# kimerein/sabatinilab-glm

Measured on NVIDIA B200. Metric: cv_model_fits_per_sec, higher is better.
Workload: dtype f64

## Files before the change

### sabatinilab-glm_b200/csrc/gram_tc.cu

```cuda
#include <cuda.h>

#include <algorithm>
#include <vector>

#include <stdlib.h>

#include "common.cuh"

namespace sglm {

constexpr int TC_SMAX = 8;
constexpr int TC_BK = 128;
constexpr int TC_BM = 256;
constexpr int TC_BN = 256;
constexpr int TC_STAGES = 3;
constexpr int TC_THREADS = 192;
constexpr int TC_MAX_KB_PER_SEG = 2048;
constexpr uint32_t TC_STAGE_BYTES = (TC_BM + TC_BN) * TC_BK;
constexpr int TC_LEAD = 64;
constexpr int TC_FAR = 1024;

__device__ __forceinline__ double z_value(const double *X, long long ldx, const double *Y, long long ldy,
                                          int C, int n_y, long long t, int c) {
    if (c < C) return X[t * ldx + c];
    if (c < C + n_y) return Y[t * ldy + (c - C)];
    return 1.0;
}

__global__ void __launch_bounds__(256)
tc_colmax_kernel(const double *__restrict__ X, long long ldx, const double *__restrict__ Y, long long ldy,
                 int C, int n_y, long long T, const double *__restrict__ rs,
                 unsigned long long *__restrict__ colmax_bits, int *__restrict__ col_lsb) {
    const int n_aug = C + n_y + 1;
    const int c = blockIdx.x * 256 + threadIdx.x;
    if (c >= n_aug) return;
    const long long rows_per = (T + gridDim.y - 1) / gridDim.y;
    const long long t0 = (long long)blockIdx.y * rows_per, t1 = min(T, t0 + rows_per);
    double m = 0.0;
    bool bad = false;
    int lsb = 0x7fffffff;
    for (long long t = t0; t < t1; ++t) {
        const double v = fabs(z_value(X, ldx, Y, ldy, C, n_y, t, c) * (rs ? rs[t] : 1.0));
        bad |= !(v <= 1.7976931348623157e308);
        m = fmax(m, v);
        const long long bits = __double_as_longlong(v);
        const int e = (int)(bits >> 52);
        const long long frac = bits & 0xfffffffffffffLL;
        if (e > 0) lsb = min(lsb, e - 1075 + __ffsll(frac | (1LL << 52)) - 1);
        else if (frac) lsb = min(lsb, -1074 + __ffsll(frac) - 1);
    }
    if (bad) m = __longlong_as_double(0x7ff8000000000000LL);
    atomicMax(colmax_bits + c, (unsigned long long)__double_as_longlong(m));
    atomicMin(col_lsb + c, lsb);
}

__device__ __forceinline__ int digits_needed(double z, int E) {
    double r = scalbn(z, -E);
    int need = 0;
    r *= 64.0;
#pragma unroll
    for (int k = 1; k <= TC_SMAX; ++k) {
        if (r == 0.0) break;
        const double d = rint(r);
        if (d != 0.0) need = k;
        r = (r - d) * 128.0;
    }
    if (r != 0.0) need = TC_SMAX;
    return need;
}

__global__ void __launch_bounds__(256)
tc_digits_kernel(const double *__restrict__ X, long long ldx, const double *__restrict__ Y, long long ldy,
                 int C, int n_y, long long T, const double *__restrict__ rs, const int *__restrict__ colE,
                 int *__restrict__ colS) {
    const int n_aug = C + n_y + 1;
    const int c = blockIdx.x * 256 + threadIdx.x;
    if (c >= n_aug) return;
    const long long rows_per = (T + gridDim.y - 1) / gridDim.y;
    const long long t0 = (long long)blockIdx.y * rows_per, t1 = min(T, t0 + rows_per);
    const int E = colE[c];
    int need = 1;
    for (long long t = t0; t < t1 && need < TC_SMAX; ++t)
        need = max(need, digits_needed(z_value(X, ldx, Y, ldy, C, n_y, t, c) * (rs ? rs[t] : 1.0), E));
    atomicMax(colS + c, need);
}

__global__ void tc_exponent_kernel(const unsigned long long *__restrict__ colmax_bits, int n_aug, int max_planes,
                                   int *__restrict__ colE, int *__restrict__ colS, int *__restrict__ flag) {
    const int c = blockIdx.x * blockDim.x + threadIdx.x;
    if (c >= n_aug) return;
    const double m = __longlong_as_double((long long)colmax_bits[c]);
    if (!(m <= 1.7976931348623157e308)) { atomicOr(flag, 1); colE[c] = 0; colS[c] = 1; return; }
    const int E = (m == 0.0) ? 0 : ilogb(m) + 1;
    colE[c] = E;
    const int lsb = colS[c];
    int need = 1;
    if (m != 0.0) {
        const int span = E - 6 - lsb;
        if (span > 0) need = 1 + (span + 6) / 7;
    }
    colS[c] = min(need, max_planes);
}

__global__ void __launch_bounds__(256)
tc_slice_kernel(const double *__restrict__ X, long long ldx, const double *__restrict__ Y, long long ldy,
                int C, int n_y, const double *__restrict__ rs, const long long *__restrict__ rows, long long n_pos,
                const int *__restrict__ colE, const int *__restrict__ colS, const int *__restrict__ plane_row,
                int8_t *__restrict__ At, long long ld_at, long long n_ident) {
    __shared__ __align__(16) double tile[32][130];
    const int n_aug = C + n_y + 1;
    const long long p0 = (long long)blockIdx.x * 128;
    const int c0 = blockIdx.y * 32;
    const int tid = threadIdx.x;
    __shared__ long long srow[128];
    if (tid < 128) srow[tid] = (p0 + tid < n_pos) ? (rows ? rows[p0 + tid] : (p0 + tid < n_ident ? p0 + tid : -1)) : -1;
    __syncthreads();
    {
        const int cc = tid & 31, c = c0 + cc;
        double v[16];
#pragma unroll
        for (int k = 0; k < 16; ++k) {
            const long long t = srow[(tid >> 5) + 8 * k];
            v[k] = (t >= 0 && c < n_aug) ? z_value(X, ldx, Y, ldy, C, n_y, t, c) * (rs ? rs[t] : 1.0) : 0.0;
        }
#pragma unroll
        for (int k = 0; k < 16; ++k) tile[cc][(tid >> 5) + 8 * k] = v[k];
    }
    __syncthreads();
    const int pq = tid & 31, cg = tid >> 5;
    const long long p = p0 + 4 * pq;
    if (p >= n_pos) return;
#pragma unroll 1
    for (int cc = cg * 4; cc < cg * 4 + 4; ++cc) {
        const int c = c0 + cc;
        if (c >= n_aug) break;
        const int S = colS[c], E = colE[c];
        const double2 v01 = *reinterpret_cast<const double2 *>(&tile[cc][4 * pq]);
        const double2 v23 = *reinterpret_cast<const double2 *>(&tile[cc][4 * pq + 2]);
        double r0, r1, r2, r3;
        if (E > -900 && E < 900) {
            const double sc = __longlong_as_double((long long)(1023 + 6 - E) << 52);
            r0 = v01.x * sc; r1 = v01.y * sc; r2 = v23.x * sc; r3 = v23.y * sc;
        } else {
            r0 = scalbn(v01.x, -E) * 64.0; r1 = scalbn(v01.y, -E) * 64.0;
            r2 = scalbn(v23.x, -E) * 64.0; r3 = scalbn(v23.y, -E) * 64.0;
        }
        for (int k = 1; k <= S; ++k) {
            const double d0 = rint(r0), d1 = rint(r1), d2 = rint(r2), d3 = rint(r3);
            r0 = (r0 - d0) * 128.0; r1 = (r1 - d1) * 128.0; r2 = (r2 - d2) * 128.0; r3 = (r3 - d3) * 128.0;
            const unsigned pack = ((unsigned)(int)d0 & 0xffu) | (((unsigned)(int)d1 & 0xffu) << 8) |
                                  (((unsigned)(int)d2 & 0xffu) << 16) | (((unsigned)(int)d3 & 0xffu) << 24);
            *reinterpret_cast<unsigned *>(At + (long long)plane_row[c * TC_SMAX + (k - 1)] * ld_at + p) = pack;
        }
    }
}

constexpr int TC_EXP_ROWS = 256;
constexpr int TC_EXP_POS = 512;
__global__ void __launch_bounds__(256)
tc_expand_kernel(const int8_t *__restrict__ Bt, long long ld_bt, const long long *__restrict__ rows, long long n_pos,
                 const int2 *__restrict__ map, int n_at_rows, int8_t *__restrict__ At, long long ld_at) {
    __shared__ long long srow[TC_EXP_POS];
    const int tid = threadIdx.x;
    const long long p0 = (long long)blockIdx.x * TC_EXP_POS;
    for (int i = tid; i < TC_EXP_POS; i += 256) srow[i] = (p0 + i < n_pos) ? rows[p0 + i] : -1;
    __syncthreads();
    const int pq = tid & 31, rl = tid >> 5;
    const long long p = p0 + 16 * pq;
    if (p >= n_pos) return;
    const long long r0 = srow[16 * pq], r15 = srow[16 * pq + 15];
    const bool contig = r0 >= 0 && r15 == r0 + 15;
    const int r_end = min(n_at_rows, (int)(blockIdx.y + 1) * TC_EXP_ROWS);
    for (int r = blockIdx.y * TC_EXP_ROWS + rl; r < r_end; r += 8) {
        const int2 m = map[r];
        if (m.x < 0) continue;
        const int8_t *src = Bt + (long long)m.x * ld_bt + m.y;
        uint4 out;
        if (contig) {
            const unsigned long long a = (unsigned long long)(src + r0);
            const unsigned *w = reinterpret_cast<const unsigned *>(a & ~3ull);
            const unsigned sh = (unsigned)(a & 3ull) * 8u;
            const unsigned w0 = __ldg(w), w1 = __ldg(w + 1), w2 = __ldg(w + 2), w3 = __ldg(w + 3);
            const unsigned w4 = sh ? __ldg(w + 4) : 0u;
            out = make_uint4(__funnelshift_r(w0, w1, sh), __funnelshift_r(w1, w2, sh), __funnelshift_r(w2, w3, sh),
                             __funnelshift_r(w3, w4, sh));
        } else {
            unsigned q[4];
#pragma unroll
            for (int j = 0; j < 4; ++j) {
                unsigned v = 0u;
#pragma unroll
                for (int b = 0; b < 4; ++b) {
                    const long long rr = srow[16 * pq + 4 * j + b];
                    if (rr >= 0) v |= (unsigned)(unsigned char)__ldg(src + rr) << (8 * b);
                }
                q[j] = v;
            }
            out = make_uint4(q[0], q[1], q[2], q[3]);
        }
        *reinterpret_cast<uint4 *>(At + (long long)r * ld_at + p) = out;
    }
}

__device__ __forceinline__ uint32_t smem_u32(const void *p) { return (uint32_t)__cvta_generic_to_shared(p); }

__device__ __forceinline__ void mbar_init(uint64_t *bar, uint32_t count) {
    asm volatile("mbarrier.init.shared::cta.b64 [%0], %1;" ::"r"(smem_u32(bar)), "r"(count));
}
__device__ __forceinline__ void mbar_expect_tx(uint64_t *bar, uint32_t bytes) {
    asm volatile("mbarrier.arrive.expect_tx.shared::cta.b64 _, [%0], %1;" ::"r"(smem_u32(bar)), "r"(bytes) : "memory");
}
__device__ __forceinline__ void mbar_arrive(uint64_t *bar) {
    asm volatile("mbarrier.arrive.shared::cta.b64 _, [%0];" ::"r"(smem_u32(bar)) : "memory");
}
__device__ __forceinline__ void mbar_wait(uint64_t *bar, uint32_t parity) {
    const uint32_t addr = smem_u32(bar);
    const long long t_start = clock64();
    while (true) {
        uint32_t done;
        asm volatile(
            "{\n\t.reg .pred p;\n\t"
            "mbarrier.try_wait.parity.shared::cta.b64 p, [%1], %2;\n\t"
            "selp.b32 %0, 1, 0, p;\n\t}"
            : "=r"(done)
            : "r"(addr), "r"(parity)
            : "memory");
        if (done) return;
        if (clock64() - t_start > 4000000000LL) { asm volatile("trap;"); }
    }
}
__device__ __forceinline__ void tma_load_2d(void *dst, const CUtensorMap *tmap, uint64_t *bar, int c0, int c1) {
    asm volatile(
        "cp.async.bulk.tensor.2d.shared::cluster.global.mbarrier::complete_tx::bytes [%0], [%1, {%3, %4}], [%2];"
        ::"r"(smem_u32(dst)), "l"((uint64_t)tmap), "r"(smem_u32(bar)), "r"(c0), "r"(c1)
        : "memory");
}
__device__ __forceinline__ void tma_load_2d_mc(void *dst, const CUtensorMap *tmap, uint64_t *bar, int c0, int c1, uint16_t mask) {
    asm volatile(
        "cp.async.bulk.tensor.2d.shared::cluster.global.mbarrier::complete_tx::bytes.multicast::cluster [%0], [%1, {%3, %4}], [%2], %5;"
        ::"r"(smem_u32(dst)), "l"((uint64_t)tmap), "r"(smem_u32(bar)), "r"(c0), "r"(c1), "h"(mask)
        : "memory");
}
__device__ __forceinline__ void tc_commit_mc(uint64_t *bar, uint16_t mask) {
    asm volatile("tcgen05.commit.cta_group::1.mbarrier::arrive::one.shared::cluster.multicast::cluster.b64 [%0], %1;"
                 ::"r"(smem_u32(bar)), "h"(mask) : "memory");
}
__device__ __forceinline__ void tc_cluster_sync() {
    asm volatile("barrier.cluster.arrive.release.aligned;\n\tbarrier.cluster.wait.acquire.aligned;" ::: "memory");
}
__device__ __forceinline__ void tc_fence_before() { asm volatile("tcgen05.fence::before_thread_sync;" ::: "memory"); }
__device__ __forceinline__ void tc_fence_after() { asm volatile("tcgen05.fence::after_thread_sync;" ::: "memory"); }
__device__ __forceinline__ void tc_commit(uint64_t *bar) {
    asm volatile("tcgen05.commit.cta_group::1.mbarrier::arrive::one.shared::cluster.b64 [%0];" ::"r"(smem_u32(bar)) : "memory");
}
__device__ __forceinline__ void tc_mma_i8(uint32_t tmem_d, uint64_t desc_a, uint64_t desc_b, uint32_t idesc, uint32_t accumulate) {
    asm volatile(
        "{\n\t.reg .pred p;\n\t"
        "setp.ne.b32 p, %4, 0;\n\t"
        "tcgen05.mma.cta_group::1.kind::i8 [%0], %1, %2, %3, p;\n\t}"
        ::"r"(tmem_d), "l"(desc_a), "l"(desc_b), "r"(idesc), "r"(accumulate)
        : "memory");
}
__device__ __forceinline__ uint64_t umma_desc_k_sw128(uint32_t smem_addr) {
    uint64_t d = 0;
    d |= (uint64_t)((smem_addr >> 4) & 0x3FFF);
    d |= (uint64_t)1 << 16;
    d |= (uint64_t)(1024 >> 4) << 32;
    d |= (uint64_t)1 << 46;
    d |= (uint64_t)2 << 61;
    return d;
}
__host__ __device__ constexpr uint32_t tc_idesc_i8() {
    return (2u << 4) | (1u << 7) | (1u << 10) | ((uint32_t)(TC_BN >> 3) << 17) | ((uint32_t)(128 >> 4) << 24);
}

struct TcSeg { int kb0, n_kb, set, first; };

__global__ void __launch_bounds__(TC_THREADS, 1)
tc_gram_i8_kernel(const __grid_constant__ CUtensorMap tmap, const int2 *__restrict__ tiles, int n_tiles,
                  int n_parts, const TcSeg *__restrict__ segs, int n_segs, long long *__restrict__ SG, long long S,
                  int *__restrict__ prog, const int2 *__restrict__ pairs, int n_pairs) {
    extern __shared__ __align__(1024) uint8_t tc_smem[];
    uint8_t *base = (uint8_t *)(((uintptr_t)tc_smem + 1023) & ~(uintptr_t)1023);
    uint8_t *sA = base;
    uint8_t *sB = base + TC_STAGES * TC_BM * TC_BK;
    uint64_t *bars = (uint64_t *)(base + TC_STAGES * TC_STAGE_BYTES);
    uint64_t *full = bars, *empty = bars + TC_STAGES, *tmem_full = bars + 2 * TC_STAGES, *tmem_empty = tmem_full + 1;
    uint32_t *tmem_slot = (uint32_t *)(tmem_empty + 1);

    const int warp = threadIdx.x >> 5, lane = threadIdx.x & 31;
    const int item = blockIdx.x;
    const int rank = item & 1;
    const int2 pr = pairs[(item >> 1) % n_pairs];
    const int part = (item >> 1) / n_pairs;
    const bool paired = pr.y >= 0;
    const int my_tile = rank == 0 ? pr.x : pr.y;
    const int2 tile = tiles[my_tile >= 0 ? my_tile : pr.x];
    const int m0 = tile.x * TC_BM, n0 = tile.y * TC_BN;
    (void)n_tiles;
    long long total_kb = 0;
    for (int sgi = 0; sgi < n_segs; ++sgi) total_kb += segs[sgi].n_kb;
    const long long part_lo = total_kb * part / n_parts, part_hi = total_kb * (part + 1) / n_parts;
    auto seg_range = [&](const TcSeg &sg, long long before, int &lo, int &hi) {
        const long long a = max(part_lo, before), b = min(part_hi, before + sg.n_kb);
        lo = sg.kb0 + (int)(a - before);
        hi = (b > a) ? sg.kb0 + (int)(b - before) : lo;
    };

    if (threadIdx.x == 0) {
        for (int s = 0; s < TC_STAGES; ++s) { mbar_init(full + s, 1); mbar_init(empty + s, paired ? 2 : 1); }
        mbar_init(tmem_full, 1);
        mbar_init(tmem_empty, 4);
        asm volatile("fence.mbarrier_init.release.cluster;" ::: "memory");
    }
    if (warp == 1) {
        asm volatile("tcgen05.alloc.cta_group::1.sync.aligned.shared::cta.b32 [%0], %1;" ::"r"(smem_u32(tmem_slot)), "r"(512));
        asm volatile("tcgen05.relinquish_alloc_permit.cta_group::1.sync.aligned;" ::);
    }
    tc_fence_before();
    __syncthreads();
    tc_cluster_sync();
    tc_fence_after();
    const uint32_t tmem_acc = *tmem_slot;
    const uint16_t mc_mask = paired ? (uint16_t)3 : (uint16_t)(1u << rank);

    if (my_tile < 0) {
        if (prog != nullptr && threadIdx.x == 0)
            asm volatile("st.relaxed.gpu.global.s32 [%0], %1;" ::"l"(prog + item), "r"(0x7fffffff) : "memory");
    } else if (warp == 0) {
        int it = 0;
        long long before = 0;
        for (int sgi = 0; sgi < n_segs; ++sgi) {
            int lo, hi;
            seg_range(segs[sgi], before, lo, hi);
            before += segs[sgi].n_kb;
            for (int kb = lo; kb < hi; ++kb, ++it) {
                if (prog != nullptr && (it & 31) == 0) {
                    __syncwarp();
                    if (lane == 0) asm volatile("st.relaxed.gpu.global.s32 [%0], %1;" ::"l"(prog + item), "r"(it) : "memory");
                    const int *grp = prog + (long long)part * 2 * n_pairs;
                    const long long t_start = clock64();
                    while (true) {
                        int behind = 0;
                        for (int j = lane; j < 2 * n_pairs; j += 32) {
                            int v;
                            asm volatile("ld.relaxed.gpu.global.s32 %0, [%1];" : "=r"(v) : "l"(grp + j) : "memory");
                            const int d = it - v;
                            if (v >= 0 && d > TC_LEAD && d <= TC_FAR) behind = 1;
                        }
                        if (!__any_sync(0xffffffffu, behind)) break;
                        __nanosleep(500);
                        if (clock64() - t_start > 4000000000LL) { asm volatile("trap;"); }
                    }
                }
                if (lane == 0) {
                    const int st = it % TC_STAGES;
                    const uint32_t ph = (it / TC_STAGES) & 1;
                    mbar_wait(empty + st, ph ^ 1);
                    mbar_expect_tx(full + st, TC_STAGE_BYTES);
                    const int kc = kb * TC_BK;
                    uint8_t *a = sA + st * TC_BM * TC_BK, *bq = sB + st * TC_BN * TC_BK;
                    if (paired) {
                        tma_load_2d_mc(a + rank * 128 * TC_BK, &tmap, full + st, kc, m0 + 128 * rank, mc_mask);
                    } else {
                        tma_load_2d(a, &tmap, full + st, kc, m0);
                        tma_load_2d(a + 128 * TC_BK, &tmap, full + st, kc, m0 + 128);
                    }
                    tma_load_2d(bq, &tmap, full + st, kc, n0);
                    tma_load_2d(bq + 128 * TC_BK, &tmap, full + st, kc, n0 + 128);
                }
            }
        }
        __syncwarp();
        if (prog != nullptr && lane == 0)
            asm volatile("st.relaxed.gpu.global.s32 [%0], %1;" ::"l"(prog + item), "r"(0x7fffffff) : "memory");
    } else if (warp == 1) {
        if (lane == 0) {
            constexpr uint32_t idesc = tc_idesc_i8();
            int it = 0, drained = 0;
            long long before = 0;
            for (int sgi = 0; sgi < n_segs; ++sgi) {
                int lo, hi;
                seg_range(segs[sgi], before, lo, hi);
                before += segs[sgi].n_kb;
                if (hi <= lo) continue;
                if (drained > 0) { mbar_wait(tmem_empty, (drained - 1) & 1); tc_fence_after(); }
                for (int kb = lo; kb < hi; ++kb, ++it) {
                    const int st = it % TC_STAGES;
                    const uint32_t ph = (it / TC_STAGES) & 1;
                    mbar_wait(full + st, ph);
                    tc_fence_after();
                    const uint64_t da0 = umma_desc_k_sw128(smem_u32(sA + st * TC_BM * TC_BK));
                    const uint64_t da1 = umma_desc_k_sw128(smem_u32(sA + st * TC_BM * TC_BK + 128 * TC_BK));
                    const uint64_t db = umma_desc_k_sw128(smem_u32(sB + st * TC_BN * TC_BK));
#pragma unroll
                    for (int k = 0; k < TC_BK / 32; ++k) {
                        const uint32_t accflag = ((kb - lo) | k) ? 1u : 0u;
                        tc_mma_i8(tmem_acc, da0 + (uint64_t)(k * 2), db + (uint64_t)(k * 2), idesc, accflag);
                        tc_mma_i8(tmem_acc + 256u, da1 + (uint64_t)(k * 2), db + (uint64_t)(k * 2), idesc, accflag);
                    }
                    if (paired) tc_commit_mc(empty + st, mc_mask);
                    else tc_commit(empty + st);
                }
                tc_commit(tmem_full);
                ++drained;
            }
        }
    } else {
        const int q = warp & 3;
        const int row = q * 32 + lane;
        int drained = 0;
        long long before = 0;
        for (int sgi = 0; sgi < n_segs; ++sgi) {
            const TcSeg sg = segs[sgi];
            int lo, hi;
            seg_range(sg, before, lo, hi);
            before += sg.n_kb;
            if (hi <= lo) continue;
            mbar_wait(tmem_full, drained & 1);
            tc_fence_after();
#pragma unroll 1
            for (int half = 0; half < 2; ++half) {
                unsigned long long *out = reinterpret_cast<unsigned long long *>(
                    SG + ((long long)sg.set * S + (m0 + half * 128 + row)) * S + n0);
#pragma unroll 1
                for (int ch = 0; ch < TC_BN / 32; ++ch) {
                    uint32_t v[32];
                    const uint32_t taddr = tmem_acc + ((uint32_t)(q * 32) << 16) + (uint32_t)(half * 256 + ch * 32);
                    asm volatile(
                        "tcgen05.ld.sync.aligned.32x32b.x32.b32 "
                        "{%0, %1, %2, %3, %4, %5, %6, %7, %8, %9, %10, %11, %12, %13, %14, %15, "
                        "%16, %17, %18, %19, %20, %21, %22, %23, %24, %25, %26, %27, %28, %29, %30, %31}, [%32];"
                        : "=r"(v[0]), "=r"(v[1]), "=r"(v[2]), "=r"(v[3]), "=r"(v[4]), "=r"(v[5]), "=r"(v[6]), "=r"(v[7]),
                          "=r"(v[8]), "=r"(v[9]), "=r"(v[10]), "=r"(v[11]), "=r"(v[12]), "=r"(v[13]), "=r"(v[14]), "=r"(v[15]),
                          "=r"(v[16]), "=r"(v[17]), "=r"(v[18]), "=r"(v[19]), "=r"(v[20]), "=r"(v[21]), "=r"(v[22]), "=r"(v[23]),
                          "=r"(v[24]), "=r"(v[25]), "=r"(v[26]), "=r"(v[27]), "=r"(v[28]), "=r"(v[29]), "=r"(v[30]), "=r"(v[31])
                        : "r"(taddr));
                    asm volatile("tcgen05.wait::ld.sync.aligned;" ::: "memory");
#pragma unroll
                    for (int j = 0; j < 32; ++j) {
                        const long long x = (long long)(int)v[j];
                        if (x != 0) atomicAdd(out + ch * 32 + j, (unsigned long long)x);
                    }
                }
            }
            tc_fence_before();
            __syncwarp();
            if (lane == 0) mbar_arrive(tmem_empty);
            ++drained;
        }
    }
    tc_fence_before();
    __syncthreads();
    tc_cluster_sync();
    if (warp == 1) {
        tc_fence_after();
        asm volatile("tcgen05.dealloc.cta_group::1.sync.aligned.b32 %0, %1;" ::"r"(tmem_acc), "r"(512));
    }
}

__global__ void __launch_bounds__(TC_THREADS, 1)
tc_mma_probe_kernel(int iters) {
    extern __shared__ __align__(1024) uint8_t tc_smem[];
    uint8_t *base = (uint8_t *)(((uintptr_t)tc_smem + 1023) & ~(uintptr_t)1023);
    uint64_t *bars = (uint64_t *)(base + TC_STAGE_BYTES);
    uint32_t *tmem_slot = (uint32_t *)(bars + 2);
    const int warp = threadIdx.x >> 5, lane = threadIdx.x & 31;
    for (int i = threadIdx.x; i < (int)(TC_STAGE_BYTES / 4); i += TC_THREADS) ((uint32_t *)base)[i] = 0x01010101u * (i & 3);
    if (threadIdx.x == 0) { mbar_init(bars, 1); asm volatile("fence.mbarrier_init.release.cluster;" ::: "memory"); }
    if (warp == 1) {
        asm volatile("tcgen05.alloc.cta_group::1.sync.aligned.shared::cta.b32 [%0], %1;" ::"r"(smem_u32(tmem_slot)), "r"(512));
        asm volatile("tcgen05.relinquish_alloc_permit.cta_group::1.sync.aligned;" ::);
    }
    asm volatile("fence.proxy.async.shared::cta;" ::: "memory");
    tc_fence_before();
    __syncthreads();
    tc_fence_after();
    const uint32_t tmem_acc = *tmem_slot;
    if (warp == 1 && lane == 0) {
        constexpr uint32_t idesc = tc_idesc_i8();
        const uint64_t da0 = umma_desc_k_sw128(smem_u32(base));
        const uint64_t da1 = umma_desc_k_sw128(smem_u32(base + 128 * TC_BK));
        const uint64_t db = umma_desc_k_sw128(smem_u32(base + TC_BM * TC_BK));
        for (int it = 0; it < iters; ++it) {
#pragma unroll
            for (int k = 0; k < TC_BK / 32; ++k) {
                tc_mma_i8(tmem_acc, da0 + (uint64_t)(k * 2), db + (uint64_t)(k * 2), idesc, (it | k) ? 1u : 0u);
                tc_mma_i8(tmem_acc + 256u, da1 + (uint64_t)(k * 2), db + (uint64_t)(k * 2), idesc, (it | k) ? 1u : 0u);
            }
        }
        tc_commit(bars);
        mbar_wait(bars, 0);
    }
    tc_fence_before();
    __syncthreads();
    if (warp == 1) {
        tc_fence_after();
        asm volatile("tcgen05.dealloc.cta_group::1.sync.aligned.b32 %0, %1;" ::"r"(tmem_acc), "r"(512));
    }
}

__global__ void __launch_bounds__(256)
tc_gram_i8_check_kernel(const int8_t *__restrict__ At, long long ld_at, const int2 *__restrict__ tiles,
                        const TcSeg *__restrict__ segs, int n_segs, long long *__restrict__ SG, long long S) {
    const int2 tile = tiles[blockIdx.x];
    const int m0 = tile.x * TC_BM, n0 = tile.y * TC_BN;
    for (int e = threadIdx.x; e < TC_BM * TC_BN; e += 256) {
        const int m = m0 + e / TC_BN, n = n0 + e % TC_BN;
        const int *a = reinterpret_cast<const int *>(At + (long long)m * ld_at);
        const int *b = reinterpret_cast<const int *>(At + (long long)n * ld_at);
        for (int sgi = 0; sgi < n_segs; ++sgi) {
            const TcSeg sg = segs[sgi];
            long long acc = 0;
            const long long i0 = (long long)sg.kb0 * (TC_BK / 4), i1 = i0 + (long long)sg.n_kb * (TC_BK / 4);
            int part = 0;
            for (long long i = i0; i < i1; ++i) {
                part = __dp4a(a[i], b[i], part);
                if ((i & 1023) == 1023) { acc += part; part = 0; }
            }
            acc += part;
            SG[((long long)sg.set * S + m) * S + n] += acc;
        }
    }
}

constexpr int TC_SUM_OUT = 8;
constexpr int TC_SUM_CELLS = 256;
__global__ void __launch_bounds__(256)
tc_zero_tiles_kernel(long long *__restrict__ SG, long long S, const int2 *__restrict__ tiles) {
    const int2 tile = tiles[blockIdx.x];
    long long *base = SG + (long long)blockIdx.y * S * S + (long long)tile.x * TC_BM * S + (long long)tile.y * TC_BN;
    for (int e = threadIdx.x; e < TC_BM * TC_BN / 2; e += 256) {
        const int r = e / (TC_BN / 2), c2 = e % (TC_BN / 2);
        reinterpret_cast<longlong2 *>(base + (long long)r * S)[c2] = make_longlong2(0, 0);
    }
}

__global__ void __launch_bounds__(256)
tc_cell_sum_kernel(const long long *__restrict__ SG, long long S, const int2 *__restrict__ tiles, int n_tiles, int n_cells,
                   const int *__restrict__ member, int n_out, long long *__restrict__ SGout) {
    __shared__ unsigned smask[TC_SUM_CELLS];
    const long long n_elem = S * S;
    const long long n_pairs = (long long)n_tiles * (TC_BM * TC_BN / 2);
    for (int o0 = 0; o0 < n_out; o0 += TC_SUM_OUT) {
        __syncthreads();
        for (int c = threadIdx.x; c < n_cells && c < TC_SUM_CELLS; c += 256) {
            unsigned m = 0;
            for (int k = 0; k < TC_SUM_OUT && o0 + k < n_out; ++k)
                if (member[(o0 + k) * n_cells + c]) m |= 1u << k;
            smask[c] = m;
        }
        __syncthreads();
        for (long long t = (long long)blockIdx.x * 256 + threadIdx.x; t < n_pairs; t += (long long)gridDim.x * 256) {
            const int2 tile = tiles[t / (TC_BM * TC_BN / 2)];
            const int w = (int)(t % (TC_BM * TC_BN / 2));
            const long long e = ((long long)tile.x * TC_BM + w / (TC_BN / 2)) * S + (long long)tile.y * TC_BN + 2 * (w % (TC_BN / 2));
            const bool two = true;
            long long a0[TC_SUM_OUT], a1[TC_SUM_OUT];
#pragma unroll
            for (int k = 0; k < TC_SUM_OUT; ++k) { a0[k] = 0; a1[k] = 0; }
#pragma unroll 4
            for (int c = 0; c < n_cells; ++c) {
                const long long *src = SG + (long long)c * n_elem + e;
                long long v0, v1 = 0;
                if (two) { const longlong2 v = *reinterpret_cast<const longlong2 *>(src); v0 = v.x; v1 = v.y; }
                else v0 = src[0];
                const unsigned m = smask[c];
#pragma unroll
                for (int k = 0; k < TC_SUM_OUT; ++k)
                    if ((m >> k) & 1u) { a0[k] += v0; a1[k] += v1; }
            }
#pragma unroll
            for (int k = 0; k < TC_SUM_OUT; ++k)
                if (o0 + k < n_out) {
                    long long *dst = SGout + (long long)(o0 + k) * n_elem + e;
                    dst[0] = a0[k];
                    if (two) dst[1] = a1[k];
                }
        }
    }
}

__global__ void __launch_bounds__(256)
tc_combine_kernel(const long long *__restrict__ SG, long long S, const int *__restrict__ colE,
                  const int *__restrict__ colS, const int *__restrict__ plane_row, int n_aug,
                  double *__restrict__ G, long long ldg) {
    const int set = blockIdx.z;
    const int c1 = blockIdx.y;
    const long long *SGs = SG + (long long)set * S * S;
    double *Gs = G + (long long)set * n_aug * ldg;
    for (int c2 = blockIdx.x * 256 + threadIdx.x; c2 < n_aug; c2 += gridDim.x * 256) {
        if (c2 < c1) continue;
        const int S1 = colS[c1], S2 = colS[c2];
        double acc = 0.0;
        for (int tot = TC_SMAX + 1; tot >= 2; --tot) {
            double part = 0.0;
            for (int k = 1; k <= S1; ++k) {
                const int l = tot - k;
                if (l < 1 || l > S2) continue;
                const int r1 = plane_row[c1 * TC_SMAX + (k - 1)], r2 = plane_row[c2 * TC_SMAX + (l - 1)];
                const long long v = (k <= l) ? SGs[(long long)r1 * S + r2] : SGs[(long long)r2 * S + r1];
                part += (double)v;
            }
            acc += scalbn(part, -(12 + 7 * (tot - 2)));
        }
        const double g = scalbn(acc, colE[c1] + colE[c2]);
        Gs[(long long)c1 * ldg + c2] = g;
        Gs[(long long)c2 * ldg + c1] = g;
    }
}

typedef CUresult (*PFN_encodeTiled)(CUtensorMap *, CUtensorMapDataType, cuuint32_t, void *, const cuuint64_t *,
                                    const cuuint64_t *, const cuuint32_t *, const cuuint32_t *,
                                    CUtensorMapInterleave, CUtensorMapSwizzle, CUtensorMapL2promotion,
                                    CUtensorMapFloatOOBfill);

static PFN_encodeTiled get_encode_fn() {
    static PFN_encodeTiled fn = nullptr;
    if (!fn) {
        void *p = nullptr;
        cudaDriverEntryPointQueryResult q;
        if (cudaGetDriverEntryPoint("cuTensorMapEncodeTiled", &p, cudaEnableDefault, &q) == cudaSuccess &&
            q == cudaDriverEntryPointSuccess)
            fn = (PFN_encodeTiled)p;
    }
    return fn;
}

}

using namespace sglm;

struct TcPlan {
    int n_aug, n_sets;
    long long S;
    long long n_pos;
    std::vector<int> plane_row;
    std::vector<int> level_off, level_cnt;
    std::vector<int2> tiles;
    std::vector<int2> pairs;
    int n_parts;
    std::vector<TcSeg> segs;
    std::vector<long long> set_pos0;
};

static void tc_make_plan(int n_aug, const int *colS, int n_sets, const long long *set_rows, TcPlan &p) {
    p.n_aug = n_aug; p.n_sets = n_sets;
    p.plane_row.assign((size_t)n_aug * TC_SMAX, -1);
    p.level_off.assign(TC_SMAX + 1, 0); p.level_cnt.assign(TC_SMAX + 1, 0);
    long long off = 0;
    for (int k = 1; k <= TC_SMAX; ++k) {
        p.level_off[k] = (int)off;
        int cnt = 0;
        for (int c = 0; c < n_aug; ++c)
            if (colS[c] >= k) p.plane_row[(size_t)c * TC_SMAX + (k - 1)] = (int)off + cnt++;
        p.level_cnt[k] = cnt;
        off += ((long long)cnt + 255) / 256 * 256;
    }
    p.S = std::max<long long>(off, 256);
    p.tiles.clear();
    for (int k = 1; k <= TC_SMAX; ++k)
        for (int l = k; l <= TC_SMAX && k + l <= TC_SMAX + 1; ++l) {
            if (!p.level_cnt[k] || !p.level_cnt[l]) continue;
            const int mt0 = p.level_off[k] / TC_BM, mt1 = (p.level_off[k] + p.level_cnt[k] + TC_BM - 1) / TC_BM;
            const int nt0 = p.level_off[l] / TC_BN, nt1 = (p.level_off[l] + p.level_cnt[l] + TC_BN - 1) / TC_BN;
            for (int mt = mt0; mt < mt1; ++mt)
                for (int nt = nt0; nt < nt1; ++nt) {
                    if (k == l && (long long)(nt + 1) * TC_BN <= (long long)mt * TC_BM) continue;
                    p.tiles.push_back(make_int2(mt, nt));
                }
        }
    p.pairs.clear();
    for (size_t i = 0; i < p.tiles.size();) {
        if (i + 1 < p.tiles.size() && p.tiles[i + 1].x == p.tiles[i].x && p.tiles[i + 1].y == p.tiles[i].y + 1) {
            p.pairs.push_back(make_int2((int)i, (int)i + 1));
            i += 2;
        } else {
            p.pairs.push_back(make_int2((int)i, -1));
            i += 1;
        }
    }
    {
        const int sms = sm_count();
        const int nt = std::max<int>(1, 2 * (int)p.pairs.size());
        long long total_kb = 0;
        for (int s = 0; s < n_sets; ++s) total_kb += (set_rows[s] + TC_BK - 1) / TC_BK;
        int best = 1;
        double best_eff = 0.0;
        for (int parts = 1; parts <= 16; ++parts) {
            if (parts > 1 && total_kb / parts < 64) break;
            const long long items = (long long)nt * parts;
            const double eff = (double)items / (double)(((items + sms - 1) / sms) * sms);
            const double score = eff - (items < 2LL * sms ? 0.5 : 0.0) - 0.002 * parts;
            if (score > best_eff) { best_eff = score; best = parts; }
        }
        p.n_parts = best;
        if (const char *v = tuning_env("SGLM_TC_PARTS")) p.n_parts = std::max(1, std::min(16, atoi(v)));
    }
    p.segs.clear(); p.set_pos0.assign(n_sets, 0);
    long long pos = 0;
    for (int s = 0; s < n_sets; ++s) {
        p.set_pos0[s] = pos;
        long long kb = (set_rows[s] + TC_BK - 1) / TC_BK;
        long long kb0 = pos / TC_BK;
        int first = 1;
        if (kb == 0) { p.segs.push_back(TcSeg{(int)kb0, 0, s, 1}); }
        while (kb > 0) {
            const int n = (int)std::min<long long>(kb, TC_MAX_KB_PER_SEG);
            p.segs.push_back(TcSeg{(int)kb0, n, s, first});
            first = 0; kb0 += n; kb -= n;
        }
        pos += (set_rows[s] + TC_BK - 1) / TC_BK * TC_BK;
    }
    p.n_pos = std::max<long long>(pos, TC_BK);
}

static inline size_t tc_align(size_t x) { return (x + 1023) & ~(size_t)1023; }

struct TcLayout { size_t off_at, off_sg, off_sgout, off_member, off_plane, off_tiles, off_segs, off_prog, off_pairs, total; };

static TcLayout tc_layout(const TcPlan &p, int n_out = 0) {
    TcLayout L;
    size_t o = 0;
    L.off_at = o; o += tc_align((size_t)p.S * p.n_pos);
    L.off_sg = o; o += tc_align((size_t)p.n_sets * p.S * p.S * sizeof(long long));
    L.off_sgout = o; o += tc_align((size_t)n_out * p.S * p.S * sizeof(long long));
    L.off_member = o; o += tc_align((size_t)n_out * p.n_sets * sizeof(int));
    L.off_plane = o; o += tc_align(p.plane_row.size() * sizeof(int));
    L.off_tiles = o; o += tc_align(p.tiles.size() * sizeof(int2));
    L.off_segs = o; o += tc_align(p.segs.size() * sizeof(TcSeg));
    L.off_prog = o; o += tc_align(2 * p.pairs.size() * (size_t)std::max(p.n_parts, 1) * sizeof(int));
    L.off_pairs = o; o += tc_align(p.pairs.size() * sizeof(int2));
    L.total = o;
    return L;
}

static void tc_lag_base_planes(int P, const int *baseS_host, std::vector<int> &bplane, int &nb) {
    bplane.assign((size_t)(P + 1) * TC_SMAX, -1);
    nb = 0;
    for (int q = 0; q <= P; ++q)
        for (int k = 0; k < std::min(std::max(baseS_host[q], 1), TC_SMAX); ++k) bplane[(size_t)q * TC_SMAX + k] = nb++;
}
struct TcLagLayout { size_t off_bt, off_bplane, off_map, total; long long ld_bt; };
static TcLagLayout tc_lag_layout(size_t base_total, int nb, int P, long long n_u, long long S) {
    TcLagLayout LL;
    LL.ld_bt = (std::max<long long>(n_u, 1) + 127) / 128 * 128;
    size_t o = tc_align(base_total);
    LL.off_bt = o; o += tc_align((size_t)nb * LL.ld_bt + 1024);
    LL.off_bplane = o; o += tc_align((size_t)(P + 1) * TC_SMAX * sizeof(int));
    LL.off_map = o; o += tc_align((size_t)S * sizeof(int2));
    LL.total = o;
    return LL;
}

static int gram_tc_analyze(const double *X, int64_t ldx, const double *Y, int64_t ldy, int32_t n_y, int64_t T,
                           int32_t C, const double *rs, int max_planes, int32_t *colE, int32_t *colS,
                           uint64_t *colmax_scratch, int32_t *flag, void *stream) {
    SGLM_CHECK_ARG(T >= 0 && C >= 0 && n_y >= 0 && ldx >= C && ldy >= n_y, SGLM_E_SHAPE, "gram_tc_analyze: bad shape");
    SGLM_CHECK_ARG(colE && colS && colmax_scratch && flag, SGLM_E_INVALID_ARG, "gram_tc_analyze: null pointer");
    cudaStream_t st = (cudaStream_t)stream;
    const int n_aug = C + n_y + 1;
    SGLM_CUDA_OK(cudaMemsetAsync(colmax_scratch, 0, (size_t)n_aug * sizeof(uint64_t), st));
    SGLM_CUDA_OK(cudaMemsetAsync(flag, 0, sizeof(int), st));
    SGLM_CUDA_OK(cudaMemsetAsync(colS, 0x7f, (size_t)n_aug * sizeof(int), st));
    const int gy = (int)std::max<long long>(1, std::min<long long>(T / 256, 64LL * sm_count() / std::max(1, ceil_div(n_aug, 256))));
    dim3 grid(ceil_div(n_aug, 256), gy);
    if (T > 0) {
        tc_colmax_kernel<<<grid, 256, 0, st>>>(X, ldx, Y, ldy, C, n_y, T, rs, (unsigned long long *)colmax_scratch, colS);
        SGLM_LAUNCH_OK("tc_colmax_kernel");
    }
    tc_exponent_kernel<<<ceil_div(n_aug, 256), 256, 0, st>>>((const unsigned long long *)colmax_scratch, n_aug, max_planes, colE, colS, flag);
    SGLM_LAUNCH_OK("tc_exponent_kernel");
    if (T > 0 && max_planes == TC_SMAX && tuning_env("SGLM_TC_DIGIT_PASS")) {
        tc_digits_kernel<<<grid, 256, 0, st>>>(X, ldx, Y, ldy, C, n_y, T, rs, colE, colS);
        SGLM_LAUNCH_OK("tc_digits_kernel");
    }
    return SGLM_OK;
}

extern "C" int sglm_gram_tc_analyze_f64(const double *X, int64_t ldx, const double *Y, int64_t ldy, int32_t n_y,
                                        int64_t T, int32_t C, int32_t *colE, int32_t *colS,
                                        uint64_t *colmax_scratch, int32_t *flag, void *stream) {
    return gram_tc_analyze(X, ldx, Y, ldy, n_y, T, C, nullptr, TC_SMAX, colE, colS, colmax_scratch, flag, stream);
}

static int gram_tc_colstats(const double *X, int64_t ldx, const double *Y, int64_t ldy, int32_t n_y, int64_t T,
                            int32_t C, const double *rs, uint64_t *colmax_bits, int32_t *col_lsb, void *stream) {
    cudaStream_t st = (cudaStream_t)stream;
    const int n_aug = C + n_y + 1;
    SGLM_CUDA_OK(cudaMemsetAsync(colmax_bits, 0, (size_t)n_aug * sizeof(uint64_t), st));
    SGLM_CUDA_OK(cudaMemsetAsync(col_lsb, 0x7f, (size_t)n_aug * sizeof(int), st));
    if (T > 0) {
        const int gy = (int)std::max<long long>(1, std::min<long long>(T / 256, 64LL * sm_count() / std::max(1, ceil_div(n_aug, 256))));
        dim3 grid(ceil_div(n_aug, 256), gy);
        tc_colmax_kernel<<<grid, 256, 0, st>>>(X, ldx, Y, ldy, C, n_y, T, rs, (unsigned long long *)colmax_bits, col_lsb);
        SGLM_LAUNCH_OK("tc_colmax_kernel");
    }
    return SGLM_OK;
}

extern "C" int sglm_gram_tc_colstats_f64(const double *X, int64_t ldx, const double *Y, int64_t ldy, int32_t n_y,
                                         int64_t T, int32_t C, uint64_t *colmax_bits, int32_t *col_lsb, void *stream) {
    SGLM_CHECK_ARG(T >= 0 && C >= 0 && n_y >= 0 && ldx >= C && ldy >= n_y, SGLM_E_SHAPE, "gram_tc_colstats: bad shape");
    SGLM_CHECK_ARG(colmax_bits && col_lsb, SGLM_E_INVALID_ARG, "gram_tc_colstats: null pointer");
    return gram_tc_colstats(X, ldx, Y, ldy, n_y, T, C, nullptr, colmax_bits, col_lsb, stream);
}

extern "C" int sglm_gram_tc_colstats_scaled_f64(const double *X, int64_t ldx, const double *Y, int64_t ldy, int32_t n_y,
                                                int64_t T, int32_t C, const double *row_scale, uint64_t *colmax_bits,
                                                int32_t *col_lsb, void *stream) {
    SGLM_CHECK_ARG(T >= 0 && C >= 0 && n_y >= 0 && ldx >= C && ldy >= n_y, SGLM_E_SHAPE, "gram_tc_colstats_scaled: bad shape");
    SGLM_CHECK_ARG(colmax_bits && col_lsb && (row_scale || T == 0), SGLM_E_INVALID_ARG, "gram_tc_colstats_scaled: null pointer");
    return gram_tc_colstats(X, ldx, Y, ldy, n_y, T, C, row_scale, colmax_bits, col_lsb, stream);
}

extern "C" int sglm_gram_tc_exponents(const uint64_t *colmax_bits, int32_t n_aug, int32_t max_planes, int32_t *colE,
                                      int32_t *colS, int32_t *flag, void *stream) {
    SGLM_CHECK_ARG(colmax_bits && colE && colS && flag && n_aug > 0, SGLM_E_INVALID_ARG, "gram_tc_exponents: bad argument");
    SGLM_CHECK_ARG(max_planes >= 1 && max_planes <= TC_SMAX, SGLM_E_INVALID_ARG, "gram_tc_exponents: max_planes out of range");
    cudaStream_t st = (cudaStream_t)stream;
    SGLM_CUDA_OK(cudaMemsetAsync(flag, 0, sizeof(int), st));
    tc_exponent_kernel<<<ceil_div(n_aug, 256), 256, 0, st>>>((const unsigned long long *)colmax_bits, n_aug, max_planes, colE, colS, flag);
    SGLM_LAUNCH_OK("tc_exponent_kernel");
    return SGLM_OK;
}

extern "C" int sglm_gram_tc_analyze_scaled_f64(const double *X, int64_t ldx, const double *Y, int64_t ldy,
                                               int32_t n_y, int64_t T, int32_t C, const double *row_scale,
                                               int32_t max_planes, int32_t *colE, int32_t *colS,
                                               uint64_t *colmax_scratch, int32_t *flag, void *stream) {
    SGLM_CHECK_ARG(max_planes >= 1 && max_planes <= TC_SMAX, SGLM_E_INVALID_ARG, "gram_tc_analyze_scaled: max_planes out of range");
    return gram_tc_analyze(X, ldx, Y, ldy, n_y, T, C, row_scale, max_planes, colE, colS, colmax_scratch, flag, stream);
}

extern "C" int sglm_probe_mma_i8(int32_t iters, int64_t *n_ctas_host, void *stream) {
    SGLM_CHECK_ARG(iters >= 1 && n_ctas_host, SGLM_E_INVALID_ARG, "probe_mma_i8: bad argument");
    const size_t smem = 1024 + (size_t)TC_STAGE_BYTES + 256;
    SGLM_CUDA_OK(cudaFuncSetAttribute(tc_mma_probe_kernel, cudaFuncAttributeMaxDynamicSharedMemorySize, (int)smem));
    const int n = sm_count();
    *n_ctas_host = n;
    tc_mma_probe_kernel<<<n, TC_THREADS, smem, (cudaStream_t)stream>>>(iters);
    SGLM_LAUNCH_OK("tc_mma_probe_kernel");
    return SGLM_OK;
}

extern "C" size_t sglm_gram_tc_workspace_bytes(int32_t n_aug, const int32_t *colS_host, int32_t n_sets,
                                               const int64_t *set_rows_host) {
    if (n_aug <= 0 || n_sets <= 0 || !colS_host || !set_rows_host) return 0;
    TcPlan p;
    tc_make_plan(n_aug, colS_host, n_sets, (const long long *)set_rows_host, p);
    return tc_layout(p).total;
}

extern "C" int sglm_gram_tc_plan_info(int32_t n_aug, const int32_t *colS_host, int32_t n_sets,
                                      const int64_t *set_rows_host, int64_t *out4) {
    SGLM_CHECK_ARG(n_aug > 0 && n_sets > 0 && colS_host && set_rows_host && out4, SGLM_E_INVALID_ARG,
                   "gram_tc_plan_info: bad argument");
    TcPlan p;
    tc_make_plan(n_aug, colS_host, n_sets, (const long long *)set_rows_host, p);
    out4[0] = p.S; out4[1] = p.n_pos; out4[2] = (int64_t)p.tiles.size(); out4[3] = (int64_t)p.n_parts;
    return SGLM_OK;
}

static int gram_tc_run(const double *X, int64_t ldx, const double *Y, int64_t ldy, int32_t n_y, int64_t T,
                       int32_t C, const int32_t *colE, const int32_t *colS, const int32_t *colS_host,
                       int32_t n_sets, const int64_t *set_rows_host, const int64_t *rows, int32_t n_out,
                       const int32_t *member_host, double *G, int64_t ldg, void *workspace, size_t workspace_bytes,
                       int32_t use_check_gemm, void *stream, const double *rs = nullptr, int stage = 0,
                       const sglm_lag_design *lag = nullptr);

extern "C" int sglm_gram_tc_f64(const double *X, int64_t ldx, const double *Y, int64_t ldy, int32_t n_y, int64_t T,
                                int32_t C, const int32_t *colE, const int32_t *colS, const int32_t *colS_host,
                                int32_t n_sets, const int64_t *set_rows_host, const int64_t *rows, double *G,
                                int64_t ldg, void *workspace, size_t workspace_bytes, int32_t use_check_gemm,
                                void *stream) {
    return gram_tc_run(X, ldx, Y, ldy, n_y, T, C, colE, colS, colS_host, n_sets, set_rows_host, rows, 0, nullptr, G, ldg,
                       workspace, workspace_bytes, use_check_gemm, stream);
}

extern "C" int sglm_gram_tc_scaled_f64(const double *X, int64_t ldx, const double *Y, int64_t ldy, int32_t n_y,
                                       int64_t T, int32_t C, const double *row_scale, const int32_t *colE,
                                       const int32_t *colS, const int32_t *colS_host, int32_t n_sets,
                                       const int64_t *set_rows_host, const int64_t *rows, double *G, int64_t ldg,
                                       void *workspace, size_t workspace_bytes, void *stream) {
    return gram_tc_run(X, ldx, Y, ldy, n_y, T, C, colE, colS, colS_host, n_sets, set_rows_host, rows, 0, nullptr, G, ldg,
                       workspace, workspace_bytes, 0, stream, row_scale);
}

extern "C" size_t sglm_gram_tc_cells_workspace_bytes(int32_t n_aug, const int32_t *colS_host, int32_t n_cells,
                                                     const int64_t *cell_rows_host, int32_t n_out) {
    if (n_aug <= 0 || n_cells <= 0 || n_out <= 0 || !colS_host || !cell_rows_host) return 0;
    TcPlan p;
    tc_make_plan(n_aug, colS_host, n_cells, (const long long *)cell_rows_host, p);
    return tc_layout(p, n_out).total;
}

extern "C" int sglm_gram_tc_cells_f64(const double *X, int64_t ldx, const double *Y, int64_t ldy, int32_t n_y,
                                      int64_t T, int32_t C, const int32_t *colE, const int32_t *colS,
                                      const int32_t *colS_host, int32_t n_cells, const int64_t *cell_rows_host,
                                      const int64_t *rows, int32_t n_out, const int32_t *member_host, double *G,
                                      int64_t ldg, void *workspace, size_t workspace_bytes, int32_t use_check_gemm,
                                      void *stream) {
    SGLM_CHECK_ARG(n_out >= 1 && member_host, SGLM_E_INVALID_ARG, "gram_tc_cells: membership table missing");
    SGLM_CHECK_ARG(n_cells <= TC_SUM_CELLS, SGLM_E_UNSUPPORTED, "gram_tc_cells: at most %d cells", TC_SUM_CELLS);
    return gram_tc_run(X, ldx, Y, ldy, n_y, T, C, colE, colS, colS_host, n_cells, cell_rows_host, rows, n_out,
                       member_host, G, ldg, workspace, workspace_bytes, use_check_gemm, stream);
}

extern "C" int sglm_gram_tc_cells_sgout(int32_t n_aug, const int32_t *colS_host, int32_t n_cells,
                                        const int64_t *cell_rows_host, int32_t n_out, uint64_t *offset_bytes,
                                        uint64_t *size_bytes) {
    SGLM_CHECK_ARG(n_aug > 0 && n_cells > 0 && n_out > 0 && colS_host && cell_rows_host && offset_bytes && size_bytes,
                   SGLM_E_INVALID_ARG, "gram_tc_cells_sgout: bad argument");
    TcPlan p;
    tc_make_plan(n_aug, colS_host, n_cells, (const long long *)cell_rows_host, p);
    const TcLayout L = tc_layout(p, n_out);
    *offset_bytes = L.off_sgout;
    *size_bytes = (uint64_t)n_out * p.S * p.S * sizeof(long long);
    return SGLM_OK;
}

extern "C" int sglm_gram_tc_cells_partial_f64(const double *X, int64_t ldx, const double *Y, int64_t ldy, int32_t n_y,
                                              int64_t T, int32_t C, const int32_t *colE, const int32_t *colS,
                                              const int32_t *colS_host, int32_t n_cells, const int64_t *cell_rows_host,
                                              const int64_t *rows, int32_t n_out, const int32_t *member_host,
                                              void *workspace, size_t workspace_bytes, void *stream) {
    SGLM_CHECK_ARG(n_out >= 1 && member_host, SGLM_E_INVALID_ARG, "gram_tc_cells_partial: membership table missing");
    SGLM_CHECK_ARG(n_cells <= TC_SUM_CELLS, SGLM_E_UNSUPPORTED, "gram_tc_cells_partial: at most %d cells", TC_SUM_CELLS);
    double dummy;
    return gram_tc_run(X, ldx, Y, ldy, n_y, T, C, colE, colS, colS_host, n_cells, cell_rows_host, rows, n_out,
                       member_host, &dummy, C + n_y + 1, workspace, workspace_bytes, 0, stream, nullptr, 1);
}

extern "C" int sglm_gram_tc_scaled_partial_f64(const double *X, int64_t ldx, const double *Y, int64_t ldy, int32_t n_y,
                                               int64_t T, int32_t C, const double *row_scale, const int32_t *colE,
                                               const int32_t *colS, const int32_t *colS_host, int32_t n_cells,
                                               const int64_t *cell_rows_host, const int64_t *rows, int32_t n_out,
                                               const int32_t *member_host, void *workspace, size_t workspace_bytes,
                                               void *stream) {
    SGLM_CHECK_ARG(n_out >= 1 && member_host, SGLM_E_INVALID_ARG, "gram_tc_scaled_partial: membership table missing");
    SGLM_CHECK_ARG(n_cells <= TC_SUM_CELLS, SGLM_E_UNSUPPORTED, "gram_tc_scaled_partial: at most %d cells", TC_SUM_CELLS);
    SGLM_CHECK_ARG(row_scale || T == 0, SGLM_E_INVALID_ARG, "gram_tc_scaled_partial: null row_scale");
    double dummy;
    return gram_tc_run(X, ldx, Y, ldy, n_y, T, C, colE, colS, colS_host, n_cells, cell_rows_host, rows, n_out,
                       member_host, &dummy, C + n_y + 1, workspace, workspace_bytes, 0, stream, row_scale, 1);
}

extern "C" int sglm_gram_tc_cells_combine_f64(int32_t C, int32_t n_y, const int32_t *colE, const int32_t *colS,
                                              const int32_t *colS_host, int32_t n_cells, const int64_t *cell_rows_host,
                                              int32_t n_out, double *G, int64_t ldg, void *workspace,
                                              size_t workspace_bytes, void *stream) {
    SGLM_CHECK_ARG(n_out >= 1, SGLM_E_INVALID_ARG, "gram_tc_cells_combine: n_out");
    static const int64_t no_rows = 0;
    return gram_tc_run(nullptr, C, nullptr, n_y, n_y, 0, C, colE, colS, colS_host, n_cells, cell_rows_host, &no_rows,
                       n_out, nullptr, G, ldg, workspace, workspace_bytes, 0, stream, nullptr, 2);
}

extern "C" size_t sglm_gram_tc_lag_workspace_bytes(int32_t n_aug, const int32_t *colS_host, int32_t n_cells,
                                                   const int64_t *cell_rows_host, int32_t n_out, int32_t P,
                                                   const int32_t *baseS_host, int64_t n_u) {
    if (n_aug <= 0 || n_cells <= 0 || n_out < 0 || !colS_host || !cell_rows_host || P <= 0 || !baseS_host || n_u < 0) return 0;
    TcPlan p;
    tc_make_plan(n_aug, colS_host, n_cells, (const long long *)cell_rows_host, p);
    std::vector<int> bplane;
    int nb = 0;
    tc_lag_base_planes(P, baseS_host, bplane, nb);
    return tc_lag_layout(tc_layout(p, n_out).total, nb, P, n_u, p.S).total;
}

extern "C" int sglm_gram_tc_lag_cells_f64(const sglm_lag_design *lag, const double *Y, int64_t ldy, int32_t n_y, int64_t T,
                                          int32_t C, const int32_t *colE, const int32_t *colS, const int32_t *colS_host,
                                          int32_t n_cells, const int64_t *cell_rows_host, const int64_t *rows,
                                          int32_t n_out, const int32_t *member_host, double *G, int64_t ldg,
                                          void *workspace, size_t workspace_bytes, int32_t partial, void *stream) {
    SGLM_CHECK_ARG(lag != nullptr, SGLM_E_INVALID_ARG, "gram_tc_lag_cells: null lag design");
    SGLM_CHECK_ARG(n_out == 0 || member_host, SGLM_E_INVALID_ARG, "gram_tc_lag_cells: membership table missing");
    SGLM_CHECK_ARG(n_out == 0 || n_cells <= TC_SUM_CELLS, SGLM_E_UNSUPPORTED, "gram_tc_lag_cells: at most %d cells", TC_SUM_CELLS);
    SGLM_CHECK_ARG(!partial || n_out > 0, SGLM_E_INVALID_ARG, "gram_tc_lag_cells: the partial form needs output sets");
    double dummy;
    return gram_tc_run(nullptr, C, Y, ldy, n_y, T, C, colE, colS, colS_host, n_cells, cell_rows_host, rows, n_out,
                       member_host, partial ? &dummy : G, partial ? (int64_t)(C + n_y + 1) : ldg, workspace, workspace_bytes, 0,
                       stream, nullptr, partial ? 1 : 0, lag);
}

static int gram_tc_run(const double *X, int64_t ldx, const double *Y, int64_t ldy, int32_t n_y, int64_t T,
                       int32_t C, const int32_t *colE, const int32_t *colS, const int32_t *colS_host,
                       int32_t n_sets, const int64_t *set_rows_host, const int64_t *rows, int32_t n_out,
                       const int32_t *member_host, double *G, int64_t ldg, void *workspace, size_t workspace_bytes,
                       int32_t use_check_gemm, void *stream, const double *rs, int stage, const sglm_lag_design *lag) {
    const int n_aug = C + n_y + 1;
    SGLM_CHECK_ARG(T >= 0 && C >= 0 && n_y >= 0 && n_sets >= 1 && ldx >= C && ldy >= n_y && ldg >= n_aug, SGLM_E_SHAPE,
                   "gram_tc: bad shape");
    SGLM_CHECK_ARG(colE && colS && colS_host && set_rows_host && rows && G && workspace, SGLM_E_INVALID_ARG,
                   "gram_tc: null pointer");
    SGLM_CHECK_ARG(((uintptr_t)workspace & 1023) == 0, SGLM_E_ALIGN, "gram_tc: workspace must be 1024-byte aligned");
    TcPlan p;
    tc_make_plan(n_aug, colS_host, n_sets, (const long long *)set_rows_host, p);
    const TcLayout L = tc_layout(p, n_out);
    SGLM_CHECK_ARG(workspace_bytes >= L.total, SGLM_E_WORKSPACE, "gram_tc: workspace too small (%zu < %zu)",
                   workspace_bytes, L.total);
    SGLM_CHECK_ARG(p.n_pos < 0x7fffffffLL && p.S < 0x7fffffffLL, SGLM_E_SHAPE, "gram_tc: problem too large");
    cudaStream_t st = (cudaStream_t)stream;
    char *ws = (char *)workspace;
    int8_t *At = (int8_t *)(ws + L.off_at);
    long long *SG = (long long *)(ws + L.off_sg);
    int *d_plane = (int *)(ws + L.off_plane);
    int2 *d_tiles = (int2 *)(ws + L.off_tiles);
    TcSeg *d_segs = (TcSeg *)(ws + L.off_segs);
    if (stage != 2) {
        long long covered = 0;
        for (int k = 1; k <= TC_SMAX; ++k) {
            const long long lo = (long long)p.level_off[k] + p.level_cnt[k];
            const long long hi = (long long)p.level_off[k] + ((long long)p.level_cnt[k] + 255) / 256 * 256;
            if (hi > lo) SGLM_CUDA_OK(cudaMemsetAsync(At + lo * p.n_pos, 0, (size_t)(hi - lo) * p.n_pos, st));
            covered = std::max(covered, hi);
        }
        if (p.S > covered) SGLM_CUDA_OK(cudaMemsetAsync(At + covered * p.n_pos, 0, (size_t)(p.S - covered) * p.n_pos, st));
    }
    if (stage != 2) {
        SGLM_CUDA_OK(cudaMemcpyAsync(d_plane, p.plane_row.data(), p.plane_row.size() * sizeof(int), cudaMemcpyHostToDevice, st));
        SGLM_CUDA_OK(cudaMemcpyAsync(d_tiles, p.tiles.data(), p.tiles.size() * sizeof(int2), cudaMemcpyHostToDevice, st));
        SGLM_CUDA_OK(cudaMemcpyAsync(ws + L.off_pairs, p.pairs.data(), p.pairs.size() * sizeof(int2), cudaMemcpyHostToDevice, st));
        SGLM_CUDA_OK(cudaMemcpyAsync(d_segs, p.segs.data(), p.segs.size() * sizeof(TcSeg), cudaMemcpyHostToDevice, st));
    }
    long long *SGout = (long long *)(ws + L.off_sgout);
    int *d_member = (int *)(ws + L.off_member);
    if (stage == 2) {
        SGLM_CUDA_OK(cudaMemcpyAsync(d_plane, p.plane_row.data(), p.plane_row.size() * sizeof(int), cudaMemcpyHostToDevice, st));
        SGLM_CUDA_OK(cudaStreamSynchronize(st));
        const long long *SGfin2 = n_out > 0 ? SGout : SG;
        const int n_fin2 = n_out > 0 ? n_out : n_sets;
        dim3 cgrid2((unsigned)std::min(ceil_div(n_aug, 256), 32), (unsigned)n_aug, (unsigned)n_fin2);
        tc_combine_kernel<<<cgrid2, 256, 0, st>>>(SGfin2, p.S, colE, colS, d_plane, n_aug, G, ldg);
        SGLM_LAUNCH_OK("tc_combine_kernel");
        return SGLM_OK;
    }
    if (n_out > 0)
        SGLM_CUDA_OK(cudaMemcpyAsync(d_member, member_host, (size_t)n_out * n_sets * sizeof(int), cudaMemcpyHostToDevice, st));
    TcLagLayout LL = {};
    std::vector<int> bplane;
    std::vector<int2> lag_map;
    if (lag) {
        SGLM_CHECK_ARG(rs == nullptr, SGLM_E_UNSUPPORTED, "gram_tc: row scales are not supported for lag designs");
        SGLM_CHECK_ARG(lag->base && lag->src_host && lag->off_host && lag->baseE && lag->baseS && lag->baseS_host &&
                       lag->P > 0 && lag->ldb >= lag->P && lag->n_u >= T, SGLM_E_INVALID_ARG, "gram_tc: bad lag design");
        int nb = 0;
        tc_lag_base_planes(lag->P, lag->baseS_host, bplane, nb);
        LL = tc_lag_layout(L.total, nb, lag->P, lag->n_u, p.S);
        SGLM_CHECK_ARG(workspace_bytes >= LL.total, SGLM_E_WORKSPACE, "gram_tc: workspace too small for the lag design (%zu < %zu)",
                       workspace_bytes, LL.total);
        lag_map.assign((size_t)p.S, make_int2(-1, 0));
        for (int c = 0; c < C; ++c) {
            const int pc = lag->src_host[c], off = lag->off_host[c];
            SGLM_CHECK_ARG(pc >= 0 && pc < lag->P && off >= 0 && (long long)off + T <= lag->n_u, SGLM_E_INVALID_ARG,
                           "gram_tc: lag column %d reads outside the base window", c);
            for (int k = 0; k < colS_host[c]; ++k) {
                const int r = p.plane_row[(size_t)c * TC_SMAX + k], b = bplane[(size_t)pc * TC_SMAX + k];
                SGLM_CHECK_ARG(r >= 0 && b >= 0, SGLM_E_INVALID_ARG, "gram_tc: lag column %d has more planes than its base signal", c);
                lag_map[(size_t)r] = make_int2(b, off);
            }
        }
        SGLM_CUDA_OK(cudaMemcpyAsync(ws + LL.off_bplane, bplane.data(), bplane.size() * sizeof(int), cudaMemcpyHostToDevice, st));
        SGLM_CUDA_OK(cudaMemcpyAsync(ws + LL.off_map, lag_map.data(), lag_map.size() * sizeof(int2), cudaMemcpyHostToDevice, st));
    }
    SGLM_CUDA_OK(cudaStreamSynchronize(st));

    if (lag) {
        int8_t *Bt = (int8_t *)(ws + LL.off_bt);
        dim3 bgrid((unsigned)(LL.ld_bt / 128), (unsigned)ceil_div(lag->P + 1, 32));
        tc_slice_kernel<<<bgrid, 256, 0, st>>>(lag->base, lag->ldb, nullptr, 0, lag->P, 0, nullptr, nullptr, LL.ld_bt, lag->baseE,
                                               lag->baseS, (const int *)(ws + LL.off_bplane), Bt, LL.ld_bt, lag->n_u);
        SGLM_LAUNCH_OK("tc_slice_kernel(base)");
        dim3 egrid((unsigned)ceil_div<long long>(p.n_pos, TC_EXP_POS), (unsigned)ceil_div((int)p.S, TC_EXP_ROWS));
        tc_expand_kernel<<<egrid, 256, 0, st>>>(Bt, LL.ld_bt, (const long long *)rows, p.n_pos, (const int2 *)(ws + LL.off_map),
                                                (int)p.S, At, p.n_pos);
        SGLM_LAUNCH_OK("tc_expand_kernel");
        dim3 ygrid((unsigned)(p.n_pos / 128), (unsigned)ceil_div(n_y + 1, 32));
        tc_slice_kernel<<<ygrid, 256, 0, st>>>(nullptr, 0, Y, ldy, 0, n_y, nullptr, (const long long *)rows, p.n_pos, colE + C,
                                               colS + C, d_plane + (size_t)C * TC_SMAX, At, p.n_pos, 0);
        SGLM_LAUNCH_OK("tc_slice_kernel(y)");
    } else {
    dim3 sgrid((unsigned)(p.n_pos / 128), (unsigned)ceil_div(n_aug, 32));
    tc_slice_kernel<<<sgrid, 256, 0, st>>>(X, ldx, Y, ldy, C, n_y, rs, (const long long *)rows, p.n_pos, colE, colS,
                                           d_plane, At, p.n_pos, 0);
    SGLM_LAUNCH_OK("tc_slice_kernel");
    }

    const int n_tiles = (int)p.tiles.size();
    if (n_tiles > 0) {
        tc_zero_tiles_kernel<<<dim3((unsigned)n_tiles, (unsigned)p.n_sets), 256, 0, st>>>(SG, p.S, d_tiles);
        SGLM_LAUNCH_OK("tc_zero_tiles_kernel");
    }
    if (use_check_gemm) {
        tc_gram_i8_check_kernel<<<n_tiles, 256, 0, st>>>(At, p.n_pos, d_tiles, d_segs, (int)p.segs.size(), SG, p.S);
        SGLM_LAUNCH_OK("tc_gram_i8_check_kernel");
    } else {
        PFN_encodeTiled enc = get_encode_fn();
        SGLM_CHECK_ARG(enc != nullptr, SGLM_E_CUDA, "gram_tc: cuTensorMapEncodeTiled not available");
        CUtensorMap tmap;
        const cuuint64_t gdim[2] = {(cuuint64_t)p.n_pos, (cuuint64_t)p.S};
        const cuuint64_t gstride[1] = {(cuuint64_t)p.n_pos};
        const cuuint32_t box[2] = {(cuuint32_t)TC_BK, 128};
        const cuuint32_t estr[2] = {1, 1};
        CUresult r = enc(&tmap, CU_TENSOR_MAP_DATA_TYPE_UINT8, 2, At, gdim, gstride, box, estr,
                         CU_TENSOR_MAP_INTERLEAVE_NONE, CU_TENSOR_MAP_SWIZZLE_128B, CU_TENSOR_MAP_L2_PROMOTION_L2_256B,
                         CU_TENSOR_MAP_FLOAT_OOB_FILL_NONE);
        SGLM_CHECK_ARG(r == CUDA_SUCCESS, SGLM_E_CUDA, "gram_tc: cuTensorMapEncodeTiled failed (%d)", (int)r);
        const size_t smem = 1024 + (size_t)TC_STAGES * TC_STAGE_BYTES + 256;
        SGLM_CUDA_OK(cudaFuncSetAttribute(tc_gram_i8_kernel, cudaFuncAttributeMaxDynamicSharedMemorySize, (int)smem));
        int *d_prog = (int *)(ws + L.off_prog);
        const bool lockstep = tuning_env("SGLM_TC_LOCKSTEP") != nullptr;
        const int n_pairs = (int)p.pairs.size();
        if (lockstep) SGLM_CUDA_OK(cudaMemsetAsync(d_prog, 0xff, (size_t)2 * n_pairs * p.n_parts * sizeof(int), st));
        cudaLaunchConfig_t cfg = {};
        cfg.gridDim = dim3((unsigned)(2 * n_pairs * p.n_parts));
        cfg.blockDim = dim3(TC_THREADS);
        cfg.dynamicSmemBytes = smem;
        cfg.stream = st;
        cudaLaunchAttribute at[1];
        at[0].id = cudaLaunchAttributeClusterDimension;
        at[0].val.clusterDim.x = 2; at[0].val.clusterDim.y = 1; at[0].val.clusterDim.z = 1;
        cfg.attrs = at;
        cfg.numAttrs = 1;
        SGLM_CUDA_OK(cudaLaunchKernelEx(&cfg, tc_gram_i8_kernel, tmap, (const int2 *)d_tiles, n_tiles, p.n_parts, (const TcSeg *)d_segs,
                                        (int)p.segs.size(), SG, (long long)p.S, lockstep ? d_prog : (int *)nullptr,
                                        (const int2 *)(ws + L.off_pairs), n_pairs));
        SGLM_LAUNCH_OK("tc_gram_i8_kernel");
    }
    const long long *SGfin = SG;
    int n_fin = n_sets;
    if (n_out > 0) {
        tc_cell_sum_kernel<<<sm_count() * 8, 256, 0, st>>>(SG, p.S, d_tiles, n_tiles, n_sets, d_member, n_out, SGout);
        SGLM_LAUNCH_OK("tc_cell_sum_kernel");
        SGfin = SGout;
        n_fin = n_out;
    }
    if (stage == 1) return SGLM_OK;
    dim3 cgrid((unsigned)std::min(ceil_div(n_aug, 256), 32), (unsigned)n_aug, (unsigned)n_fin);
    tc_combine_kernel<<<cgrid, 256, 0, st>>>(SGfin, p.S, colE, colS, d_plane, n_aug, G, ldg);
    SGLM_LAUNCH_OK("tc_combine_kernel");
    return SGLM_OK;
}
```

Measured before the change: 4286.

## Route lag designs through a shifted-base correlation GEMM with scatter into Gram

Adds a lag-design path that builds shifted copies of the base signal, computes lagged cross-correlations with the int8 tcgen05 GEMM via per-k-block positions, bounding boxes and single-half A tiles, and scatters them into the Gram tiles. Signed segments let one correlation be subtracted, and the expanded-design construction is skipped when this path is taken. The goal is to avoid materialising and multiplying the full lag-expanded design matrix. The cost is considerably more kernel and host planning complexity, plus scatter kernels whose reads are uncoalesced.

```diff
diff --git a/sabatinilab-glm_b200/csrc/gram_tc.cu b/sabatinilab-glm_b200/csrc/gram_tc.cu
--- a/sabatinilab-glm_b200/csrc/gram_tc.cu
+++ b/sabatinilab-glm_b200/csrc/gram_tc.cu
@@ -202,6 +202,118 @@
     }
 }
 
+__global__ void __launch_bounds__(256)
+tc_run_starts_kernel(const long long *__restrict__ rows, long long n_pos, const long long *__restrict__ cell_pos0, int n_cells,
+                     int *__restrict__ count, longlong2 *__restrict__ out) {
+    const long long p = (long long)blockIdx.x * 256 + threadIdx.x;
+    if (p >= n_pos) return;
+    const long long r = rows[p];
+    if (r < 0) return;
+    bool start = p == 0 || rows[p - 1] < 0 || rows[p - 1] != r - 1;
+    if (!start && (p % TC_BK) == 0)
+        for (int c = 0; c < n_cells; ++c) start |= cell_pos0[c] == p;
+    if (start) out[atomicAdd(count, 1)] = make_longlong2(p, r);
+}
+
+__global__ void __launch_bounds__(256)
+tc_shift_copies_kernel(int8_t *__restrict__ W, long long n) {
+    const long long e = ((long long)blockIdx.x * 256 + threadIdx.x) * 16;
+    if (e >= n) return;
+    const uint4 lo = *reinterpret_cast<const uint4 *>(W + e);
+    const uint4 hi = e + 16 < n ? *reinterpret_cast<const uint4 *>(W + e + 16) : make_uint4(0u, 0u, 0u, 0u);
+    const unsigned w[8] = {lo.x, lo.y, lo.z, lo.w, hi.x, hi.y, hi.z, hi.w};
+#pragma unroll
+    for (int j = 1; j < 16; ++j) {
+        const int q = j >> 2;
+        const unsigned sh = (unsigned)(j & 3) * 8u;
+        const uint4 out = make_uint4(__funnelshift_r(w[q], w[q + 1], sh), __funnelshift_r(w[q + 1], w[q + 2], sh),
+                                     __funnelshift_r(w[q + 2], w[q + 3], sh), __funnelshift_r(w[q + 3], w[q + 4], sh));
+        *reinterpret_cast<uint4 *>(W + (long long)j * n + e) = out;
+    }
+}
+
+struct TcPiece { int pos0, s0, len, theta; };
+constexpr int TC_PIECE_ROWS = 1024;
+__global__ void __launch_bounds__(256)
+tc_expand_pieces_kernel(const int8_t *__restrict__ W, long long ld_w, const TcPiece *__restrict__ pieces, int n_pieces,
+                        long long n_pos, const int2 *__restrict__ map, int n_at_rows, int8_t *__restrict__ At) {
+    __shared__ int ss[TC_EXP_POS], sth[TC_EXP_POS];
+    const int tid = threadIdx.x;
+    const long long p0 = (long long)blockIdx.x * TC_EXP_POS;
+    for (int i = tid; i < TC_EXP_POS; i += 256) {
+        const long long p = p0 + i;
+        int lo = 0, hi = n_pieces;
+        while (lo < hi) { const int mid = (lo + hi) >> 1; if (pieces[mid].pos0 <= p) lo = mid + 1; else hi = mid; }
+        int s = 0, th = 0x7fffffff;
+        if (lo > 0) {
+            const TcPiece q = pieces[lo - 1];
+            if (p < (long long)q.pos0 + q.len) { s = q.s0 + (int)(p - q.pos0); th = q.theta; }
+        }
+        ss[i] = s; sth[i] = th;
+    }
+    __syncthreads();
+    const int pq = tid & 31, rl = tid >> 5;
+    const long long p = p0 + 16 * pq;
+    if (p >= n_pos) return;
+    const int s_first = ss[16 * pq], th_first = sth[16 * pq];
+    const bool one_piece = sth[16 * pq + 15] == th_first && ss[16 * pq + 15] == s_first + 15 && th_first != 0x7fffffff;
+    const int r_end = min(n_at_rows, (int)(blockIdx.y + 1) * TC_PIECE_ROWS);
+    for (int r = blockIdx.y * TC_PIECE_ROWS + rl; r < r_end; r += 8) {
+        const int2 m = map[r];
+        uint4 out = make_uint4(0u, 0u, 0u, 0u);
+        if (m.x >= 0 && !(one_piece && s_first + 15 + m.y < th_first)) {
+            const int8_t *src = W + (long long)m.x * ld_w + m.y;
+            if (one_piece && s_first + m.y >= th_first) {
+                const unsigned long long a = (unsigned long long)(src + s_first);
+                const unsigned *w = reinterpret_cast<const unsigned *>(a & ~3ull);
+                const unsigned sh = (unsigned)(a & 3ull) * 8u;
+                const unsigned w0 = __ldg(w), w1 = __ldg(w + 1), w2 = __ldg(w + 2), w3 = __ldg(w + 3);
+                const unsigned w4 = sh ? __ldg(w + 4) : 0u;
+                out = make_uint4(__funnelshift_r(w0, w1, sh), __funnelshift_r(w1, w2, sh), __funnelshift_r(w2, w3, sh),
+                                 __funnelshift_r(w3, w4, sh));
+            } else {
+                unsigned q[4];
+#pragma unroll
+                for (int j = 0; j < 4; ++j) {
+                    unsigned v = 0u;
+#pragma unroll
+                    for (int b = 0; b < 4; ++b) {
+                        const int i = 16 * pq + 4 * j + b;
+                        if (sth[i] != 0x7fffffff && ss[i] + m.y >= sth[i])
+                            v |= (unsigned)(unsigned char)__ldg(src + ss[i]) << (8 * b);
+                    }
+                    q[j] = v;
+                }
+                out = make_uint4(q[0], q[1], q[2], q[3]);
+            }
+        }
+        *reinterpret_cast<uint4 *>(At + (long long)r * n_pos + p) = out;
+    }
+}
+
+__global__ void __launch_bounds__(256)
+tc_corr_scatter_kernel(const long long *__restrict__ Corr, long long rows_c, long long ld_c, int n_lag,
+                       const int2 *__restrict__ map, long long *__restrict__ SG, long long S, const int2 *__restrict__ tiles) {
+    __shared__ int2 mr[TC_BM], mc[TC_BN];
+    const int2 tile = tiles[blockIdx.x];
+    const int cell = blockIdx.y;
+    for (int i = threadIdx.x; i < TC_BM; i += 256) mr[i] = map[tile.x * TC_BM + i];
+    for (int i = threadIdx.x; i < TC_BN; i += 256) mc[i] = map[tile.y * TC_BN + i];
+    __syncthreads();
+    const long long *Cc = Corr + (long long)cell * rows_c * ld_c;
+    long long *base = SG + (long long)cell * S * S + (long long)tile.x * TC_BM * S + (long long)tile.y * TC_BN;
+    for (int e = threadIdx.x; e < TC_BM * TC_BN; e += 256) {
+        const int r = e / TC_BN, c = e % TC_BN;
+        int2 a = mr[r], b = mc[c];
+        long long v = 0;
+        if (a.x >= 0 && b.x >= 0) {
+            if (a.y > b.y) { const int2 t = a; a = b; b = t; }
+            v = Cc[(long long)a.x * ld_c + ((long long)(b.x >> 7) * n_lag + (b.y - a.y)) * 128 + (b.x & 127)];
+        }
+        base[(long long)r * S + c] = v;
+    }
+}
+
 __device__ __forceinline__ uint32_t smem_u32(const void *p) { return (uint32_t)__cvta_generic_to_shared(p); }
 
 __device__ __forceinline__ void mbar_init(uint64_t *bar, uint32_t count) {
@@ -274,12 +386,13 @@
     return (2u << 4) | (1u << 7) | (1u << 10) | ((uint32_t)(TC_BN >> 3) << 17) | ((uint32_t)(128 >> 4) << 24);
 }
 
-struct TcSeg { int kb0, n_kb, set, first; };
+struct TcSeg { int kb0, n_kb, set, neg; };
 
 __global__ void __launch_bounds__(TC_THREADS, 1)
 tc_gram_i8_kernel(const __grid_constant__ CUtensorMap tmap, const int2 *__restrict__ tiles, int n_tiles,
-                  int n_parts, const TcSeg *__restrict__ segs, int n_segs, long long *__restrict__ SG, long long S,
-                  int *__restrict__ prog, const int2 *__restrict__ pairs, int n_pairs) {
+                  int n_parts, const TcSeg *__restrict__ segs, int n_segs, long long *__restrict__ SG, long long ld_out,
+                  long long rows_out, int *__restrict__ prog, const int2 *__restrict__ pairs, int n_pairs,
+                  const int *__restrict__ kpos, const int4 *__restrict__ bbox, int a_halves) {
     extern __shared__ __align__(1024) uint8_t tc_smem[];
     uint8_t *base = (uint8_t *)(((uintptr_t)tc_smem + 1023) & ~(uintptr_t)1023);
     uint8_t *sA = base;
@@ -357,17 +470,23 @@
                     const int st = it % TC_STAGES;
                     const uint32_t ph = (it / TC_STAGES) & 1;
                     mbar_wait(empty + st, ph ^ 1);
-                    mbar_expect_tx(full + st, TC_STAGE_BYTES);
-                    const int kc = kb * TC_BK;
+                    mbar_expect_tx(full + st, TC_STAGE_BYTES - (2 - a_halves) * 128 * TC_BK);
+                    const int kc = kpos ? (kpos[kb] & ~15) : kb * TC_BK;
                     uint8_t *a = sA + st * TC_BM * TC_BK, *bq = sB + st * TC_BN * TC_BK;
                     if (paired) {
-                        tma_load_2d_mc(a + rank * 128 * TC_BK, &tmap, full + st, kc, m0 + 128 * rank, mc_mask);
+                        if (rank < a_halves) tma_load_2d_mc(a + rank * 128 * TC_BK, &tmap, full + st, kc, m0 + 128 * rank, mc_mask);
                     } else {
                         tma_load_2d(a, &tmap, full + st, kc, m0);
-                        tma_load_2d(a + 128 * TC_BK, &tmap, full + st, kc, m0 + 128);
+                        if (a_halves == 2) tma_load_2d(a + 128 * TC_BK, &tmap, full + st, kc, m0 + 128);
                     }
-                    tma_load_2d(bq, &tmap, full + st, kc, n0);
-                    tma_load_2d(bq + 128 * TC_BK, &tmap, full + st, kc, n0 + 128);
+                    if (bbox) {
+                        const int4 bb = bbox[tile.y];
+                        tma_load_2d(bq, &tmap, full + st, kc + bb.y, bb.x);
+                        tma_load_2d(bq + 128 * TC_BK, &tmap, full + st, kc + bb.w, bb.z);
+                    } else {
+                        tma_load_2d(bq, &tmap, full + st, kc, n0);
+                        tma_load_2d(bq + 128 * TC_BK, &tmap, full + st, kc, n0 + 128);
+                    }
                 }
             }
         }
@@ -393,11 +512,11 @@
                     const uint64_t da0 = umma_desc_k_sw128(smem_u32(sA + st * TC_BM * TC_BK));
                     const uint64_t da1 = umma_desc_k_sw128(smem_u32(sA + st * TC_BM * TC_BK + 128 * TC_BK));
                     const uint64_t db = umma_desc_k_sw128(smem_u32(sB + st * TC_BN * TC_BK));
-#pragma unroll
-                    for (int k = 0; k < TC_BK / 32; ++k) {
+                    const int nsub = kpos ? (kpos[kb] & 3) + 1 : TC_BK / 32;
+                    for (int k = 0; k < nsub; ++k) {
                         const uint32_t accflag = ((kb - lo) | k) ? 1u : 0u;
                         tc_mma_i8(tmem_acc, da0 + (uint64_t)(k * 2), db + (uint64_t)(k * 2), idesc, accflag);
-                        tc_mma_i8(tmem_acc + 256u, da1 + (uint64_t)(k * 2), db + (uint64_t)(k * 2), idesc, accflag);
+                        if (a_halves == 2) tc_mma_i8(tmem_acc + 256u, da1 + (uint64_t)(k * 2), db + (uint64_t)(k * 2), idesc, accflag);
                     }
                     if (paired) tc_commit_mc(empty + st, mc_mask);
                     else tc_commit(empty + st);
@@ -420,9 +539,9 @@
             mbar_wait(tmem_full, drained & 1);
             tc_fence_after();
 #pragma unroll 1
-            for (int half = 0; half < 2; ++half) {
+            for (int half = 0; half < a_halves; ++half) {
                 unsigned long long *out = reinterpret_cast<unsigned long long *>(
-                    SG + ((long long)sg.set * S + (m0 + half * 128 + row)) * S + n0);
+                    SG + ((long long)sg.set * rows_out + (m0 + half * 128 + row)) * ld_out + n0);
 #pragma unroll 1
                 for (int ch = 0; ch < TC_BN / 32; ++ch) {
                     uint32_t v[32];
@@ -440,7 +559,7 @@
 #pragma unroll
                     for (int j = 0; j < 32; ++j) {
                         const long long x = (long long)(int)v[j];
-                        if (x != 0) atomicAdd(out + ch * 32 + j, (unsigned long long)x);
+                        if (x != 0) atomicAdd(out + ch * 32 + j, (unsigned long long)(sg.neg ? -x : x));
                     }
                 }
             }
@@ -644,6 +763,43 @@
     std::vector<long long> set_pos0;
 };
 
+static void tc_push_segs(std::vector<TcSeg> &segs, long long kb0, long long n_kb, int set, int neg) {
+    while (n_kb > 0) {
+        const int n = (int)std::min<long long>(n_kb, TC_MAX_KB_PER_SEG);
+        segs.push_back(TcSeg{(int)kb0, n, set, neg});
+        kb0 += n; n_kb -= n;
+    }
+}
+
+static std::vector<int2> tc_pair_tiles(const std::vector<int2> &tiles) {
+    std::vector<int2> pairs;
+    for (size_t i = 0; i < tiles.size();) {
+        if (i + 1 < tiles.size() && tiles[i + 1].x == tiles[i].x && tiles[i + 1].y == tiles[i].y + 1) {
+            pairs.push_back(make_int2((int)i, (int)i + 1));
+            i += 2;
+        } else {
+            pairs.push_back(make_int2((int)i, -1));
+            i += 1;
+        }
+    }
+    return pairs;
+}
+
+static int tc_pick_parts(int n_ctas, long long total_kb, int max_parts) {
+    const int sms = sm_count();
+    const int nt = std::max(1, n_ctas);
+    int best = 1;
+    double best_eff = 0.0;
+    for (int parts = 1; parts <= max_parts; ++parts) {
+        if (parts > 1 && total_kb / parts < 64) break;
+        const long long items = (long long)nt * parts;
+        const double eff = (double)items / (double)(((items + sms - 1) / sms) * sms);
+        const double score = eff - (items < 2LL * sms ? 0.5 : 0.0) - 0.002 * parts;
+        if (score > best_eff) { best_eff = score; best = parts; }
+    }
+    return best;
+}
+
 static void tc_make_plan(int n_aug, const int *colS, int n_sets, const long long *set_rows, TcPlan &p) {
     p.n_aug = n_aug; p.n_sets = n_sets;
     p.plane_row.assign((size_t)n_aug * TC_SMAX, -1);
@@ -670,31 +826,11 @@
                     p.tiles.push_back(make_int2(mt, nt));
                 }
         }
-    p.pairs.clear();
-    for (size_t i = 0; i < p.tiles.size();) {
-        if (i + 1 < p.tiles.size() && p.tiles[i + 1].x == p.tiles[i].x && p.tiles[i + 1].y == p.tiles[i].y + 1) {
-            p.pairs.push_back(make_int2((int)i, (int)i + 1));
-            i += 2;
-        } else {
-            p.pairs.push_back(make_int2((int)i, -1));
-            i += 1;
-        }
-    }
+    p.pairs = tc_pair_tiles(p.tiles);
     {
-        const int sms = sm_count();
-        const int nt = std::max<int>(1, 2 * (int)p.pairs.size());
         long long total_kb = 0;
         for (int s = 0; s < n_sets; ++s) total_kb += (set_rows[s] + TC_BK - 1) / TC_BK;
-        int best = 1;
-        double best_eff = 0.0;
-        for (int parts = 1; parts <= 16; ++parts) {
-            if (parts > 1 && total_kb / parts < 64) break;
-            const long long items = (long long)nt * parts;
-            const double eff = (double)items / (double)(((items + sms - 1) / sms) * sms);
-            const double score = eff - (items < 2LL * sms ? 0.5 : 0.0) - 0.002 * parts;
-            if (score > best_eff) { best_eff = score; best = parts; }
-        }
-        p.n_parts = best;
+        p.n_parts = tc_pick_parts(2 * (int)p.pairs.size(), total_kb, 16);
         if (const char *v = tuning_env("SGLM_TC_PARTS")) p.n_parts = std::max(1, std::min(16, atoi(v)));
     }
     p.segs.clear(); p.set_pos0.assign(n_sets, 0);
@@ -703,16 +839,44 @@
         p.set_pos0[s] = pos;
         long long kb = (set_rows[s] + TC_BK - 1) / TC_BK;
         long long kb0 = pos / TC_BK;
-        int first = 1;
-        if (kb == 0) { p.segs.push_back(TcSeg{(int)kb0, 0, s, 1}); }
-        while (kb > 0) {
-            const int n = (int)std::min<long long>(kb, TC_MAX_KB_PER_SEG);
-            p.segs.push_back(TcSeg{(int)kb0, n, s, first});
-            first = 0; kb0 += n; kb -= n;
-        }
+        if (kb == 0) { p.segs.push_back(TcSeg{(int)kb0, 0, s, 0}); }
+        tc_push_segs(p.segs, kb0, kb, s, 0);
         pos += (set_rows[s] + TC_BK - 1) / TC_BK * TC_BK;
     }
     p.n_pos = std::max<long long>(pos, TC_BK);
+}
+
+static int tc_launch_gemm(const int8_t *tensor, long long ld, long long rows, const int2 *d_tiles, int n_tiles,
+                          const int2 *d_pairs, int n_pairs, int n_parts, const TcSeg *d_segs, int n_segs, long long *out,
+                          long long ld_out, long long rows_out, int *d_prog, const int *d_kpos, const int4 *d_bbox,
+                          int a_halves, cudaStream_t st) {
+    PFN_encodeTiled enc = get_encode_fn();
+    SGLM_CHECK_ARG(enc != nullptr, SGLM_E_CUDA, "gram_tc: cuTensorMapEncodeTiled not available");
+    CUtensorMap tmap;
+    const cuuint64_t gdim[2] = {(cuuint64_t)ld, (cuuint64_t)rows};
+    const cuuint64_t gstride[1] = {(cuuint64_t)ld};
+    const cuuint32_t box[2] = {(cuuint32_t)TC_BK, 128};
+    const cuuint32_t estr[2] = {1, 1};
+    CUresult r = enc(&tmap, CU_TENSOR_MAP_DATA_TYPE_UINT8, 2, (void *)tensor, gdim, gstride, box, estr,
+                     CU_TENSOR_MAP_INTERLEAVE_NONE, CU_TENSOR_MAP_SWIZZLE_128B, CU_TENSOR_MAP_L2_PROMOTION_L2_256B,
+                     CU_TENSOR_MAP_FLOAT_OOB_FILL_NONE);
+    SGLM_CHECK_ARG(r == CUDA_SUCCESS, SGLM_E_CUDA, "gram_tc: cuTensorMapEncodeTiled failed (%d)", (int)r);
+    const size_t smem = 1024 + (size_t)TC_STAGES * TC_STAGE_BYTES + 256;
+    SGLM_CUDA_OK(cudaFuncSetAttribute(tc_gram_i8_kernel, cudaFuncAttributeMaxDynamicSharedMemorySize, (int)smem));
+    cudaLaunchConfig_t cfg = {};
+    cfg.gridDim = dim3((unsigned)(2 * n_pairs * n_parts));
+    cfg.blockDim = dim3(TC_THREADS);
+    cfg.dynamicSmemBytes = smem;
+    cfg.stream = st;
+    cudaLaunchAttribute at[1];
+    at[0].id = cudaLaunchAttributeClusterDimension;
+    at[0].val.clusterDim.x = 2; at[0].val.clusterDim.y = 1; at[0].val.clusterDim.z = 1;
+    cfg.attrs = at;
+    cfg.numAttrs = 1;
+    SGLM_CUDA_OK(cudaLaunchKernelEx(&cfg, tc_gram_i8_kernel, tmap, d_tiles, n_tiles, n_parts, d_segs, n_segs, out, ld_out,
+                                    rows_out, d_prog, d_pairs, n_pairs, d_kpos, d_bbox, a_halves));
+    SGLM_LAUNCH_OK("tc_gram_i8_kernel");
+    return SGLM_OK;
 }
 
 static inline size_t tc_align(size_t x) { return (x + 1023) & ~(size_t)1023; }
@@ -981,6 +1145,208 @@
     return gram_tc_run(nullptr, C, Y, ldy, n_y, T, C, colE, colS, colS_host, n_cells, cell_rows_host, rows, n_out,
                        member_host, partial ? &dummy : G, partial ? (int64_t)(C + n_y + 1) : ldg, workspace, workspace_bytes, 0,
                        stream, nullptr, partial ? 1 : 0, lag);
+}
+
+constexpr int TC_CORR_SHIFTS = 16;
+struct TcCorrPlan {
+    int dmax = 0, n_lag = 1, nw = 0, nmt = 0, nnt = 0;
+    long long n_pos = 0;
+    std::vector<TcPiece> pieces;
+    std::vector<int> kpos;
+    std::vector<TcSeg> csegs, gsegs;
+    int n_runs = 0, n_corr_runs = 0;
+};
+
+static int tc_corr_plan(const std::vector<std::vector<longlong2>> &runs, int dmax, long long T, long long n_u,
+                        TcCorrPlan &cp) {
+    cp.dmax = dmax; cp.n_lag = dmax + 1;
+    const long long r_min = 2LL * dmax + TC_BK;
+    cp.pieces.clear(); cp.kpos.clear(); cp.csegs.clear(); cp.gsegs.clear();
+    cp.n_runs = cp.n_corr_runs = 0;
+    long long pos = 0;
+    for (size_t c = 0; c < runs.size(); ++c) {
+        long long kb_c0 = (long long)cp.kpos.size();
+        std::vector<TcPiece> neg;
+        const long long pos_c0 = pos;
+        for (const longlong2 &rn : runs[c]) {
+            const long long a = rn.x, len = rn.y, b = a + len;
+            SGLM_CHECK_ARG(a >= 0 && len > 0 && b <= T, SGLM_E_SHAPE, "gram_tc: run [%lld, %lld) outside the %lld design rows", a, b, T);
+            ++cp.n_runs;
+            if (len < r_min) {
+                cp.pieces.push_back(TcPiece{(int)pos, (int)a, (int)len, (int)a});
+                pos += len;
+                continue;
+            }
+            ++cp.n_corr_runs;
+            const long long a0 = a & ~15LL;
+            long long g = a0 + (b - a0) / TC_BK * TC_BK;
+            for (long long kc = a0; kc < g; kc += TC_BK) {
+                SGLM_CHECK_ARG(kc >= 0 && kc + dmax + TC_BK <= n_u, SGLM_E_SHAPE,
+                               "gram_tc: core block at %lld reads past the %lld window rows", kc, n_u);
+                cp.kpos.push_back((int)kc | 3);
+            }
+            const long long nsub = (b - g) / 32;
+            if (nsub > 0 && g + dmax + TC_BK <= n_u) {
+                cp.kpos.push_back((int)g | (int)(nsub - 1));
+                g += 32 * nsub;
+            }
+            SGLM_CHECK_ARG(b - 1 + dmax < n_u, SGLM_E_SHAPE, "gram_tc: run edge reads past the window");
+            cp.pieces.push_back(TcPiece{(int)pos, (int)(g - dmax), (int)(b - g + dmax), (int)g});
+            pos += b - g + dmax;
+            neg.push_back(TcPiece{0, (int)(a0 - dmax), (int)(a - a0 + dmax), (int)a0});
+        }
+        tc_push_segs(cp.csegs, kb_c0, (long long)cp.kpos.size() - kb_c0, (int)c, 0);
+        pos = (pos + TC_BK - 1) / TC_BK * TC_BK;
+        tc_push_segs(cp.gsegs, pos_c0 / TC_BK, (pos - pos_c0) / TC_BK, (int)c, 0);
+        const long long neg0 = pos;
+        for (TcPiece q : neg) { q.pos0 = (int)pos; cp.pieces.push_back(q); pos += q.len; }
+        pos = (pos + TC_BK - 1) / TC_BK * TC_BK;
+        tc_push_segs(cp.gsegs, neg0 / TC_BK, (pos - neg0) / TC_BK, (int)c, 1);
+        SGLM_CHECK_ARG(pos < 0x7fffffffLL, SGLM_E_SHAPE, "gram_tc: problem too large");
+    }
+    cp.n_pos = std::max<long long>(pos, TC_BK);
+    return SGLM_OK;
+}
+
+static int tc_lag_corr_route(const sglm_lag_design *lag, const double *Y, int64_t ldy, int32_t n_y, int64_t T, int32_t C,
+                             const int32_t *colE, const int32_t *colS, const int32_t *colS_host, const int64_t *set_rows_host,
+                             const int64_t *rows, const TcPlan &p, const TcLayout &L, const TcLagLayout &LL, int nb,
+                             std::vector<int2> wmap, long long *SG, char *ws, cudaStream_t st, bool *taken) {
+    *taken = false;
+    const int n_cells = p.n_sets;
+    int dmax = 0;
+    for (int c = 0; c < C; ++c) dmax = std::max(dmax, lag->off_host[c]);
+    const long long r_min = 2LL * dmax + TC_BK;
+    bool any = false;
+    for (int c = 0; c < n_cells; ++c) any |= (c + 1 < n_cells ? p.set_pos0[c + 1] - p.set_pos0[c] : p.n_pos - p.set_pos0[c]) >= r_min;
+    if (!any || lag->n_u >= 0x7fffff00LL) return SGLM_OK;
+    char *at_region = ws + L.off_at;
+    const size_t at_bytes = tc_align((size_t)p.S * p.n_pos);
+    int *d_count = (int *)at_region;
+    longlong2 *d_starts = (longlong2 *)(at_region + 1024);
+    long long *d_pos0 = (long long *)(at_region + 1024 + tc_align((size_t)p.n_pos * sizeof(longlong2)));
+    SGLM_CUDA_OK(cudaMemsetAsync(d_count, 0, sizeof(int), st));
+    SGLM_CUDA_OK(cudaMemcpyAsync(d_pos0, p.set_pos0.data(), (size_t)n_cells * sizeof(long long), cudaMemcpyHostToDevice, st));
+    tc_run_starts_kernel<<<(unsigned)ceil_div<long long>(p.n_pos, 256), 256, 0, st>>>((const long long *)rows, p.n_pos, d_pos0,
+                                                                                      n_cells, d_count, d_starts);
+    SGLM_LAUNCH_OK("tc_run_starts_kernel");
+    int n_starts = 0;
+    SGLM_CUDA_OK(cudaMemcpyAsync(&n_starts, d_count, sizeof(int), cudaMemcpyDeviceToHost, st));
+    SGLM_CUDA_OK(cudaStreamSynchronize(st));
+    std::vector<longlong2> starts((size_t)n_starts);
+    if (n_starts > 0)
+        SGLM_CUDA_OK(cudaMemcpyAsync(starts.data(), d_starts, (size_t)n_starts * sizeof(longlong2), cudaMemcpyDeviceToHost, st));
+    SGLM_CUDA_OK(cudaStreamSynchronize(st));
+    std::sort(starts.begin(), starts.end(), [](const longlong2 &u, const longlong2 &v) { return u.x < v.x; });
+    std::vector<std::vector<longlong2>> runs((size_t)n_cells);
+    {
+        int c = 0;
+        for (size_t i = 0; i < starts.size(); ++i) {
+            const long long q = starts[i].x;
+            while (c + 1 < n_cells && p.set_pos0[c + 1] <= q) ++c;
+            long long end = (i + 1 < starts.size()) ? starts[i + 1].x : p.n_pos;
+            if (c + 1 < n_cells) end = std::min<long long>(end, p.set_pos0[c + 1]);
+            runs[(size_t)c].push_back(make_longlong2(starts[i].y, end - q));
+        }
+    }
+    for (int c = 0; c < n_cells; ++c) {
+        long long left = set_rows_host[c];
+        for (longlong2 &rn : runs[(size_t)c]) { rn.y = std::min(rn.y, left); left -= rn.y; }
+    }
+    TcCorrPlan cp;
+    int rc = tc_corr_plan(runs, dmax, T, lag->n_u, cp);
+    if (rc != SGLM_OK) return rc;
+    if (cp.n_corr_runs == 0) return SGLM_OK;
+    std::vector<int> yplane((size_t)(n_y + 1) * TC_SMAX, -1);
+    int nw = nb;
+    for (int j = 0; j <= n_y; ++j)
+        for (int k = 0; k < colS_host[C + j]; ++k) {
+            const int r = p.plane_row[(size_t)(C + j) * TC_SMAX + k];
+            yplane[(size_t)j * TC_SMAX + k] = nw;
+            wmap[(size_t)r] = make_int2(nw++, 0);
+        }
+    cp.nw = nw;
+    cp.nmt = ceil_div(nw, TC_BM);
+    const int nrb = ceil_div(nw, 128);
+    const long long nw_pad = 128LL * nrb;
+    const int n_boxes = nrb * cp.n_lag;
+    cp.nnt = ceil_div(n_boxes, 2);
+    std::vector<int4> bbox((size_t)cp.nnt);
+    auto box = [&](int bi, int &row, int &shift) {
+        const int rb = bi / cp.n_lag, d = bi % cp.n_lag;
+        row = (int)((d % TC_CORR_SHIFTS) * nw_pad) + rb * 128;
+        shift = d - d % TC_CORR_SHIFTS;
+    };
+    for (int nt = 0; nt < cp.nnt; ++nt) {
+        const int b0 = 2 * nt, b1 = std::min(2 * nt + 1, n_boxes - 1);
+        int4 bb;
+        box(b0, bb.x, bb.y);
+        box(b1, bb.z, bb.w);
+        bbox[(size_t)nt] = bb;
+    }
+    std::vector<int2> ctiles;
+    for (int mt = 0; mt < cp.nmt; ++mt)
+        for (int nt = 0; nt < cp.nnt; ++nt) ctiles.push_back(make_int2(mt, nt));
+    const std::vector<int2> cpairs = tc_pair_tiles(ctiles);
+    const int cparts = tc_pick_parts(2 * (int)cpairs.size(), (long long)cp.kpos.size(), 64);
+    const int gparts = tc_pick_parts(2 * (int)p.pairs.size(), cp.n_pos / TC_BK, 16);
+    const int a_halves = nw <= 128 ? 1 : 2;
+    const long long rows_c = (long long)cp.nmt * 128 * a_halves, ld_c = (long long)cp.nnt * TC_BN;
+    size_t o = 0;
+    auto take = [&](size_t bytes) { const size_t at = o; o += tc_align(bytes); return at; };
+    const size_t o_w = take((size_t)TC_CORR_SHIFTS * nw_pad * LL.ld_bt), o_corr = take((size_t)n_cells * rows_c * ld_c * sizeof(long long));
+    const size_t o_pieces = take(cp.pieces.size() * sizeof(TcPiece)), o_kpos = take(cp.kpos.size() * sizeof(int));
+    const size_t o_bbox = take(bbox.size() * sizeof(int4)), o_csegs = take(cp.csegs.size() * sizeof(TcSeg));
+    const size_t o_gsegs = take(cp.gsegs.size() * sizeof(TcSeg)), o_ctiles = take(ctiles.size() * sizeof(int2));
+    const size_t o_cpairs = take(cpairs.size() * sizeof(int2)), o_yplane = take(yplane.size() * sizeof(int));
+    const size_t o_at = take((size_t)p.S * cp.n_pos);
+    if (o > at_bytes) return SGLM_OK;
+    *taken = true;
+    int8_t *W = (int8_t *)(at_region + o_w);
+    long long *Corr = (long long *)(at_region + o_corr);
+    int8_t *At = (int8_t *)(at_region + o_at);
+    auto up = [&](size_t off, const void *src, size_t bytes) {
+        return bytes ? cudaMemcpyAsync(at_region + off, src, bytes, cudaMemcpyHostToDevice, st) : cudaSuccess;
+    };
+    SGLM_CUDA_OK(up(o_pieces, cp.pieces.data(), cp.pieces.size() * sizeof(TcPiece)));
+    SGLM_CUDA_OK(up(o_kpos, cp.kpos.data(), cp.kpos.size() * sizeof(int)));
+    SGLM_CUDA_OK(up(o_bbox, bbox.data(), bbox.size() * sizeof(int4)));
+    SGLM_CUDA_OK(up(o_csegs, cp.csegs.data(), cp.csegs.size() * sizeof(TcSeg)));
+    SGLM_CUDA_OK(up(o_gsegs, cp.gsegs.data(), cp.gsegs.size() * sizeof(TcSeg)));
+    SGLM_CUDA_OK(up(o_ctiles, ctiles.data(), ctiles.size() * sizeof(int2)));
+    SGLM_CUDA_OK(up(o_cpairs, cpairs.data(), cpairs.size() * sizeof(int2)));
+    SGLM_CUDA_OK(up(o_yplane, yplane.data(), yplane.size() * sizeof(int)));
+    SGLM_CUDA_OK(cudaMemcpyAsync(ws + LL.off_map, wmap.data(), wmap.size() * sizeof(int2), cudaMemcpyHostToDevice, st));
+    SGLM_CUDA_OK(cudaStreamSynchronize(st));
+    if (nw_pad > nw) SGLM_CUDA_OK(cudaMemsetAsync(W + (size_t)nw * LL.ld_bt, 0, (size_t)(nw_pad - nw) * LL.ld_bt, st));
+    dim3 bgrid((unsigned)(LL.ld_bt / 128), (unsigned)ceil_div(lag->P + 1, 32));
+    tc_slice_kernel<<<bgrid, 256, 0, st>>>(lag->base, lag->ldb, nullptr, 0, lag->P, 0, nullptr, nullptr, LL.ld_bt, lag->baseE,
+                                           lag->baseS, (const int *)(ws + LL.off_bplane), W, LL.ld_bt, lag->n_u);
+    SGLM_LAUNCH_OK("tc_slice_kernel(base)");
+    dim3 ygrid((unsigned)(LL.ld_bt / 128), (unsigned)ceil_div(n_y + 1, 32));
+    tc_slice_kernel<<<ygrid, 256, 0, st>>>(nullptr, 0, Y, ldy, 0, n_y, nullptr, nullptr, LL.ld_bt, colE + C, colS + C,
+                                           (const int *)(at_region + o_yplane), W, LL.ld_bt, T);
+    SGLM_LAUNCH_OK("tc_slice_kernel(y)");
+    const long long n_chunks = nw_pad * LL.ld_bt / 16;
+    tc_shift_copies_kernel<<<(unsigned)ceil_div<long long>(n_chunks, 256), 256, 0, st>>>(W, nw_pad * LL.ld_bt);
+    SGLM_LAUNCH_OK("tc_shift_copies_kernel");
+    SGLM_CUDA_OK(cudaMemsetAsync(Corr, 0, (size_t)n_cells * rows_c * ld_c * sizeof(long long), st));
+    rc = tc_launch_gemm(W, LL.ld_bt, TC_CORR_SHIFTS * nw_pad, (const int2 *)(at_region + o_ctiles), (int)ctiles.size(),
+                        (const int2 *)(at_region + o_cpairs), (int)cpairs.size(), cparts, (const TcSeg *)(at_region + o_csegs),
+                        (int)cp.csegs.size(), Corr, ld_c, rows_c, nullptr, (const int *)(at_region + o_kpos),
+                        (const int4 *)(at_region + o_bbox), a_halves, st);
+    if (rc != SGLM_OK) return rc;
+    const int n_tiles = (int)p.tiles.size();
+    const int2 *d_tiles = (const int2 *)(ws + L.off_tiles);
+    tc_corr_scatter_kernel<<<dim3((unsigned)n_tiles, (unsigned)n_cells), 256, 0, st>>>(Corr, rows_c, ld_c, cp.n_lag,
+                                                                                       (const int2 *)(ws + LL.off_map), SG, p.S, d_tiles);
+    SGLM_LAUNCH_OK("tc_corr_scatter_kernel");
+    dim3 egrid((unsigned)ceil_div<long long>(cp.n_pos, TC_EXP_POS), (unsigned)ceil_div((int)p.S, TC_PIECE_ROWS));
+    tc_expand_pieces_kernel<<<egrid, 256, 0, st>>>(W, LL.ld_bt, (const TcPiece *)(at_region + o_pieces), (int)cp.pieces.size(),
+                                                   cp.n_pos, (const int2 *)(ws + LL.off_map), (int)p.S, At);
+    SGLM_LAUNCH_OK("tc_expand_pieces_kernel");
+    return tc_launch_gemm(At, cp.n_pos, p.S, d_tiles, n_tiles, (const int2 *)(ws + L.off_pairs), (int)p.pairs.size(), gparts,
+                          (const TcSeg *)(at_region + o_gsegs), (int)cp.gsegs.size(), SG, p.S, p.S, nullptr, nullptr, nullptr, 2, st);
 }
 
 static int gram_tc_run(const double *X, int64_t ldx, const double *Y, int64_t ldy, int32_t n_y, int64_t T,
@@ -1008,16 +1374,6 @@
     int2 *d_tiles = (int2 *)(ws + L.off_tiles);
     TcSeg *d_segs = (TcSeg *)(ws + L.off_segs);
     if (stage != 2) {
-        long long covered = 0;
-        for (int k = 1; k <= TC_SMAX; ++k) {
-            const long long lo = (long long)p.level_off[k] + p.level_cnt[k];
-            const long long hi = (long long)p.level_off[k] + ((long long)p.level_cnt[k] + 255) / 256 * 256;
-            if (hi > lo) SGLM_CUDA_OK(cudaMemsetAsync(At + lo * p.n_pos, 0, (size_t)(hi - lo) * p.n_pos, st));
-            covered = std::max(covered, hi);
-        }
-        if (p.S > covered) SGLM_CUDA_OK(cudaMemsetAsync(At + covered * p.n_pos, 0, (size_t)(p.S - covered) * p.n_pos, st));
-    }
-    if (stage != 2) {
         SGLM_CUDA_OK(cudaMemcpyAsync(d_plane, p.plane_row.data(), p.plane_row.size() * sizeof(int), cudaMemcpyHostToDevice, st));
         SGLM_CUDA_OK(cudaMemcpyAsync(d_tiles, p.tiles.data(), p.tiles.size() * sizeof(int2), cudaMemcpyHostToDevice, st));
         SGLM_CUDA_OK(cudaMemcpyAsync(ws + L.off_pairs, p.pairs.data(), p.pairs.size() * sizeof(int2), cudaMemcpyHostToDevice, st));
@@ -1040,11 +1396,11 @@
     TcLagLayout LL = {};
     std::vector<int> bplane;
     std::vector<int2> lag_map;
+    int nb = 0;
     if (lag) {
         SGLM_CHECK_ARG(rs == nullptr, SGLM_E_UNSUPPORTED, "gram_tc: row scales are not supported for lag designs");
         SGLM_CHECK_ARG(lag->base && lag->src_host && lag->off_host && lag->baseE && lag->baseS && lag->baseS_host &&
                        lag->P > 0 && lag->ldb >= lag->P && lag->n_u >= T, SGLM_E_INVALID_ARG, "gram_tc: bad lag design");
-        int nb = 0;
         tc_lag_base_planes(lag->P, lag->baseS_host, bplane, nb);
         LL = tc_lag_layout(L.total, nb, lag->P, lag->n_u, p.S);
         SGLM_CHECK_ARG(workspace_bytes >= LL.total, SGLM_E_WORKSPACE, "gram_tc: workspace too small for the lag design (%zu < %zu)",
@@ -1065,67 +1421,58 @@
     }
     SGLM_CUDA_OK(cudaStreamSynchronize(st));
 
+    const int n_tiles = (int)p.tiles.size();
+    bool corr_route = false;
     if (lag) {
-        int8_t *Bt = (int8_t *)(ws + LL.off_bt);
-        dim3 bgrid((unsigned)(LL.ld_bt / 128), (unsigned)ceil_div(lag->P + 1, 32));
-        tc_slice_kernel<<<bgrid, 256, 0, st>>>(lag->base, lag->ldb, nullptr, 0, lag->P, 0, nullptr, nullptr, LL.ld_bt, lag->baseE,
-                                               lag->baseS, (const int *)(ws + LL.off_bplane), Bt, LL.ld_bt, lag->n_u);
-        SGLM_LAUNCH_OK("tc_slice_kernel(base)");
-        dim3 egrid((unsigned)ceil_div<long long>(p.n_pos, TC_EXP_POS), (unsigned)ceil_div((int)p.S, TC_EXP_ROWS));
-        tc_expand_kernel<<<egrid, 256, 0, st>>>(Bt, LL.ld_bt, (const long long *)rows, p.n_pos, (const int2 *)(ws + LL.off_map),
-                                                (int)p.S, At, p.n_pos);
-        SGLM_LAUNCH_OK("tc_expand_kernel");
-        dim3 ygrid((unsigned)(p.n_pos / 128), (unsigned)ceil_div(n_y + 1, 32));
-        tc_slice_kernel<<<ygrid, 256, 0, st>>>(nullptr, 0, Y, ldy, 0, n_y, nullptr, (const long long *)rows, p.n_pos, colE + C,
-                                               colS + C, d_plane + (size_t)C * TC_SMAX, At, p.n_pos, 0);
-        SGLM_LAUNCH_OK("tc_slice_kernel(y)");
-    } else {
-    dim3 sgrid((unsigned)(p.n_pos / 128), (unsigned)ceil_div(n_aug, 32));
-    tc_slice_kernel<<<sgrid, 256, 0, st>>>(X, ldx, Y, ldy, C, n_y, rs, (const long long *)rows, p.n_pos, colE, colS,
-                                           d_plane, At, p.n_pos, 0);
-    SGLM_LAUNCH_OK("tc_slice_kernel");
-    }
-
-    const int n_tiles = (int)p.tiles.size();
-    if (n_tiles > 0) {
-        tc_zero_tiles_kernel<<<dim3((unsigned)n_tiles, (unsigned)p.n_sets), 256, 0, st>>>(SG, p.S, d_tiles);
-        SGLM_LAUNCH_OK("tc_zero_tiles_kernel");
-    }
-    if (use_check_gemm) {
-        tc_gram_i8_check_kernel<<<n_tiles, 256, 0, st>>>(At, p.n_pos, d_tiles, d_segs, (int)p.segs.size(), SG, p.S);
-        SGLM_LAUNCH_OK("tc_gram_i8_check_kernel");
-    } else {
-        PFN_encodeTiled enc = get_encode_fn();
-        SGLM_CHECK_ARG(enc != nullptr, SGLM_E_CUDA, "gram_tc: cuTensorMapEncodeTiled not available");
-        CUtensorMap tmap;
-        const cuuint64_t gdim[2] = {(cuuint64_t)p.n_pos, (cuuint64_t)p.S};
-        const cuuint64_t gstride[1] = {(cuuint64_t)p.n_pos};
-        const cuuint32_t box[2] = {(cuuint32_t)TC_BK, 128};
-        const cuuint32_t estr[2] = {1, 1};
-        CUresult r = enc(&tmap, CU_TENSOR_MAP_DATA_TYPE_UINT8, 2, At, gdim, gstride, box, estr,
-                         CU_TENSOR_MAP_INTERLEAVE_NONE, CU_TENSOR_MAP_SWIZZLE_128B, CU_TENSOR_MAP_L2_PROMOTION_L2_256B,
-                         CU_TENSOR_MAP_FLOAT_OOB_FILL_NONE);
-        SGLM_CHECK_ARG(r == CUDA_SUCCESS, SGLM_E_CUDA, "gram_tc: cuTensorMapEncodeTiled failed (%d)", (int)r);
-        const size_t smem = 1024 + (size_t)TC_STAGES * TC_STAGE_BYTES + 256;
-        SGLM_CUDA_OK(cudaFuncSetAttribute(tc_gram_i8_kernel, cudaFuncAttributeMaxDynamicSharedMemorySize, (int)smem));
-        int *d_prog = (int *)(ws + L.off_prog);
-        const bool lockstep = tuning_env("SGLM_TC_LOCKSTEP") != nullptr;
-        const int n_pairs = (int)p.pairs.size();
-        if (lockstep) SGLM_CUDA_OK(cudaMemsetAsync(d_prog, 0xff, (size_t)2 * n_pairs * p.n_parts * sizeof(int), st));
-        cudaLaunchConfig_t cfg = {};
-        cfg.gridDim = dim3((unsigned)(2 * n_pairs * p.n_parts));
-        cfg.blockDim = dim3(TC_THREADS);
-        cfg.dynamicSmemBytes = smem;
-        cfg.stream = st;
-        cudaLaunchAttribute at[1];
-        at[0].id = cudaLaunchAttributeClusterDimension;
-        at[0].val.clusterDim.x = 2; at[0].val.clusterDim.y = 1; at[0].val.clusterDim.z = 1;
-        cfg.attrs = at;
-        cfg.numAttrs = 1;
-        SGLM_CUDA_OK(cudaLaunchKernelEx(&cfg, tc_gram_i8_kernel, tmap, (const int2 *)d_tiles, n_tiles, p.n_parts, (const TcSeg *)d_segs,
-                                        (int)p.segs.size(), SG, (long long)p.S, lockstep ? d_prog : (int *)nullptr,
-                                        (const int2 *)(ws + L.off_pairs), n_pairs));
-        SGLM_LAUNCH_OK("tc_gram_i8_kernel");
+        const int rc = tc_lag_corr_route(lag, Y, ldy, n_y, T, C, colE, colS, colS_host, set_rows_host, rows, p, L, LL, nb, lag_map,
+                                         SG, ws, st, &corr_route);
+        if (rc != SGLM_OK) return rc;
+    }
+    if (!corr_route) {
+        long long covered = 0;
+        for (int k = 1; k <= TC_SMAX; ++k) {
+            const long long lo = (long long)p.level_off[k] + p.level_cnt[k];
+            const long long hi = (long long)p.level_off[k] + ((long long)p.level_cnt[k] + 255) / 256 * 256;
+            if (hi > lo) SGLM_CUDA_OK(cudaMemsetAsync(At + lo * p.n_pos, 0, (size_t)(hi - lo) * p.n_pos, st));
+            covered = std::max(covered, hi);
+        }
+        if (p.S > covered) SGLM_CUDA_OK(cudaMemsetAsync(At + covered * p.n_pos, 0, (size_t)(p.S - covered) * p.n_pos, st));
+        if (lag) {
+            int8_t *Bt = (int8_t *)(ws + LL.off_bt);
+            dim3 bgrid((unsigned)(LL.ld_bt / 128), (unsigned)ceil_div(lag->P + 1, 32));
+            tc_slice_kernel<<<bgrid, 256, 0, st>>>(lag->base, lag->ldb, nullptr, 0, lag->P, 0, nullptr, nullptr, LL.ld_bt, lag->baseE,
+                                                   lag->baseS, (const int *)(ws + LL.off_bplane), Bt, LL.ld_bt, lag->n_u);
+            SGLM_LAUNCH_OK("tc_slice_kernel(base)");
+            dim3 egrid((unsigned)ceil_div<long long>(p.n_pos, TC_EXP_POS), (unsigned)ceil_div((int)p.S, TC_EXP_ROWS));
+            tc_expand_kernel<<<egrid, 256, 0, st>>>(Bt, LL.ld_bt, (const long long *)rows, p.n_pos, (const int2 *)(ws + LL.off_map),
+                                                    (int)p.S, At, p.n_pos);
+            SGLM_LAUNCH_OK("tc_expand_kernel");
+            dim3 ygrid((unsigned)(p.n_pos / 128), (unsigned)ceil_div(n_y + 1, 32));
+            tc_slice_kernel<<<ygrid, 256, 0, st>>>(nullptr, 0, Y, ldy, 0, n_y, nullptr, (const long long *)rows, p.n_pos, colE + C,
+                                                   colS + C, d_plane + (size_t)C * TC_SMAX, At, p.n_pos, 0);
+            SGLM_LAUNCH_OK("tc_slice_kernel(y)");
+        } else {
+            dim3 sgrid((unsigned)(p.n_pos / 128), (unsigned)ceil_div(n_aug, 32));
+            tc_slice_kernel<<<sgrid, 256, 0, st>>>(X, ldx, Y, ldy, C, n_y, rs, (const long long *)rows, p.n_pos, colE, colS,
+                                                   d_plane, At, p.n_pos, 0);
+            SGLM_LAUNCH_OK("tc_slice_kernel");
+        }
+        if (n_tiles > 0) {
+            tc_zero_tiles_kernel<<<dim3((unsigned)n_tiles, (unsigned)p.n_sets), 256, 0, st>>>(SG, p.S, d_tiles);
+            SGLM_LAUNCH_OK("tc_zero_tiles_kernel");
+        }
+        if (use_check_gemm) {
+            tc_gram_i8_check_kernel<<<n_tiles, 256, 0, st>>>(At, p.n_pos, d_tiles, d_segs, (int)p.segs.size(), SG, p.S);
+            SGLM_LAUNCH_OK("tc_gram_i8_check_kernel");
+        } else {
+            int *d_prog = (int *)(ws + L.off_prog);
+            const bool lockstep = tuning_env("SGLM_TC_LOCKSTEP") != nullptr;
+            const int n_pairs = (int)p.pairs.size();
+            if (lockstep) SGLM_CUDA_OK(cudaMemsetAsync(d_prog, 0xff, (size_t)2 * n_pairs * p.n_parts * sizeof(int), st));
+            const int rc = tc_launch_gemm(At, p.n_pos, p.S, d_tiles, n_tiles, (const int2 *)(ws + L.off_pairs), n_pairs, p.n_parts,
+                                          d_segs, (int)p.segs.size(), SG, p.S, p.S, lockstep ? d_prog : nullptr, nullptr, nullptr, 2, st);
+            if (rc != SGLM_OK) return rc;
+        }
     }
     const long long *SGfin = SG;
     int n_fin = n_sets;
```

Result: faster. 4456, median of 6 (+4.0%).
